# mkpython3/Mutation-Simulator

Hardware: AMD Instinct MI355X
Metric: Mbases mutated/sec on 3 Gb synthetic genome, ARGS SNP rate 0.01 (higher is better)
Workload: dtype u8

## Files before the change

include/msim.h:

```cpp
#ifndef MSIM_H
#define MSIM_H

#include <stdint.h>

#ifdef __cplusplus
extern "C" {
#endif

#define MSIM_ABI_VERSION 8

#define MSIM_OK               0
#define MSIM_ERR_ARG          1
#define MSIM_ERR_HIP          2
#define MSIM_ERR_VALUE        3
#define MSIM_ERR_KEY          4
#define MSIM_ERR_UNSUPPORTED  5
#define MSIM_ERR_NOMEM        6
#define MSIM_ERR_IO           7

#define MSIM_SN  1
#define MSIM_IN  2
#define MSIM_DE  3
#define MSIM_DU  4
#define MSIM_IV  5
// ... 182 lines not shown
#define MSIM_FASTA_HAS_BODY    1u
#define MSIM_FASTA_BAD_LINES   2u
#define MSIM_FASTA_NONUNIFORM  4u
typedef struct msim_fasta_record {
    uint64_t h0, h1;
    uint64_t b0, b1;
    uint64_t n_bases;
    uint32_t lenc, lenb;
    uint32_t flags, rsv;
} msim_fasta_record;
int msim_fasta_index(const uint8_t *text, uint64_t n, msim_fasta_record *records, uint64_t cap, uint64_t *n_records);

#define MSIM_COMM_ID_BYTES 128
int msim_comm_unique_id(uint8_t id[MSIM_COMM_ID_BYTES]);
int msim_comm_init(msim_ctx *ctx, const uint8_t id[MSIM_COMM_ID_BYTES], int rank, int world);
int msim_comm_destroy(msim_ctx *ctx);
int msim_planned_out_len(msim_ctx *ctx, int contig, uint64_t *out_len, int *known);
int msim_gather_to_root(msim_ctx *ctx, int n, const int *contig_ids, const int *owner, const uint64_t *out_len,
                        const uint64_t *n_records, const uint64_t *pool_len, int root, uint64_t *device_addrs);
int msim_gather_plan(int n, const int *owner, const uint64_t *out_len, const uint64_t *n_records, const uint64_t *pool_len,
                     int rank, int world, int root, int64_t *ops, int *n_ops);
int msim_gather_fetch(msim_ctx *ctx, uint64_t device_addr, uint64_t bytes, void *dst);

#define MSIM_SPECTRUM_TILE 4096
int msim_context_counts(msim_ctx *ctx, int contig, uint64_t counts[64], uint64_t *n_valid);
int msim_plan_contig_spectrum(msim_ctx *ctx, int contig, const uint64_t thr[192], uint64_t key, uint32_t seq);
int msim_spectrum_timing(msim_ctx *ctx, double *census_ms, double *plan_ms);
int msim_dbg_context_counts(const uint8_t *bases, uint64_t L, uint64_t counts[64], uint64_t *n_valid);
int msim_dbg_spectrum_plan(const uint8_t *bases, uint64_t L, const uint64_t thr[192], uint64_t key, uint32_t seq,
                           msim_record *recs, uint64_t cap, uint64_t *n_recs);
#define MSIM_SBS_CHANNELS 96
#define MSIM_SBS_TALLIES   8
#define MSIM_SBS_PASS   1024
int msim_sbs_counts(msim_ctx *ctx, int contig, uint64_t channels[96], uint64_t tallies[8]);
int msim_sbs_timing(msim_ctx *ctx, double *kernel_ms);
int msim_dbg_sbs_counts(const uint8_t *bases, uint64_t L, const msim_record *recs, uint64_t n_records,
                        uint64_t channels[96], uint64_t tallies[8]);

#define MSIM_CMP_EXACT  1u
#define MSIM_CMP_BINS   5
#define MSIM_CMP_PASS   256
#define MSIM_CMP_WINDOW 65536
int msim_cmp_hold(msim_ctx *ctx, int contig);
int msim_cmp_release(msim_ctx *ctx, int contig);
int msim_cmp_counts(msim_ctx *ctx, int contig, uint32_t flags, uint64_t *counts, uint64_t tallies[2]);
int msim_cmp_fetch(msim_ctx *ctx, int contig, uint64_t *n_held, uint64_t *held_pool_len, msim_record *held, uint8_t *held_pool,
                   uint8_t *held_flags, uint8_t *current_flags);
int msim_cmp_timing(msim_ctx *ctx, double *kernel_ms);
int msim_dbg_cmp_counts(const uint8_t *bases, uint64_t L, const msim_record *truth, uint64_t n_truth, const uint8_t *truth_pool,
                        uint64_t truth_pool_len, const msim_record *calls, uint64_t n_calls, const uint8_t *calls_pool,
                        uint64_t calls_pool_len, uint32_t flags, uint64_t *counts, uint64_t tallies[2], uint8_t *truth_flags,
                        uint8_t *calls_flags);

#define MSIM_CMP_BLOCK_GAP     50
#define MSIM_CMP_BLOCK_RECORDS 64
#define MSIM_CMP_BLOCK_SPAN    4096
int msim_cmp_counts_blocks(msim_ctx *ctx, int contig, uint32_t flags, uint32_t gap, uint64_t *counts, uint64_t tallies[2],
                           uint64_t block_tallies[5]);
int msim_cmp_blocks_timing(msim_ctx *ctx, double *kernel_ms);
int msim_dbg_cmp_counts_blocks(const uint8_t *bases, uint64_t L, const msim_record *truth, uint64_t n_truth, const uint8_t *truth_pool,
                               uint64_t truth_pool_len, const msim_record *calls, uint64_t n_calls, const uint8_t *calls_pool,
                               uint64_t calls_pool_len, uint32_t flags, uint32_t gap, uint64_t *counts, uint64_t tallies[2],
                               uint64_t block_tallies[5], uint8_t *truth_flags, uint8_t *calls_flags);

#define MSIM_CMP_TRUTH 0
#define MSIM_CMP_CALLS 1
#define MSIM_CMP_JOIN_TILE 1024
int msim_cmp_join(msim_ctx *ctx, int contig, int side);
int msim_cmp_counts_diploid(msim_ctx *ctx, int contig, uint32_t flags, uint64_t *counts, uint64_t tallies[2]);
int msim_cmp_fetch_diploid(msim_ctx *ctx, int contig, int side, uint64_t *n, uint64_t *pool_len, msim_record *recs, uint8_t *pool,
                           uint8_t *gt, uint8_t *flags);
int msim_cmp_join_timing(msim_ctx *ctx, double *kernel_ms);
int msim_dbg_cmp_join(const msim_record *h1, uint64_t n1, const uint8_t *pool1, uint64_t pool1_len, const msim_record *h2, uint64_t n2,
                      const uint8_t *pool2, uint64_t pool2_len, msim_record *out, uint8_t *out_pool, uint8_t *out_gt, uint64_t *n_out);
int msim_dbg_cmp_counts_diploid(const uint8_t *bases, uint64_t L, const msim_record *truth, uint64_t n_truth, const uint8_t *truth_pool,
                                uint64_t truth_pool_len, const uint8_t *truth_gt, const msim_record *calls, uint64_t n_calls,
                                const uint8_t *calls_pool, uint64_t calls_pool_len, const uint8_t *calls_gt, uint32_t flags,
                                uint64_t *counts, uint64_t tallies[2], uint8_t *truth_flags, uint8_t *calls_flags);

#define MSIM_SNP_BLOCK_WORDS 8192
int msim_dbg_snp_draws(msim_ctx *ctx, const uint32_t *words, uint64_t n_words, uint64_t ti_lim, uint64_t start, uint32_t K,
                       uint32_t aux_off, uint32_t *lanes, uint32_t *maps, uint64_t *end_pos, uint32_t *flags, uint8_t *aux);

int msim_stats(msim_ctx *ctx, msim_timing *out);
int msim_reset_stats(msim_ctx *ctx);

#ifdef __cplusplus
}
#endif
#endif
```

mutation-simulator_amd/csrc/apply.hip:

```cpp
#include <algorithm>
#include <vector>

#include "ctx.h"

#ifndef MSIM_ABL
#define MSIM_ABL 0
#endif

namespace msim {

namespace {

constexpr int THREADS = 256;
constexpr int GROUP = 16;
#ifndef MSIM_ITERS
#define MSIM_ITERS 4
#endif
constexpr int ITERS = MSIM_ITERS;
constexpr int TILE = THREADS * GROUP * ITERS;
constexpr int REC_CAP = 1024;
constexpr int REC_CAP_SMALL = 35 * ITERS;
constexpr int SCAN_ITEMS = 4;
constexpr int SCAN_BLOCK = THREADS * SCAN_ITEMS;

// ... 746 lines not shown
    } else {
        for (uint64_t i = i0; i < len; i++) dst[i] = (uint8_t)(w[(i - i0) >> 2] >> (((i - i0) & 3) * 8));
    }
}

__global__ __launch_bounds__(THREADS) void k_checksum(const uint8_t *__restrict__ src, uint64_t len,
                                                      unsigned long long *__restrict__ sum) {
    const uint64_t nwords = (len + 7) / 8;
    unsigned long long acc = 0;
    for (uint64_t k = (uint64_t)blockIdx.x * THREADS + threadIdx.x; k < nwords; k += (uint64_t)gridDim.x * THREADS) {
        uint64_t w;
        if (k * 8 + 8 <= len) {
            w = *reinterpret_cast<const uint64_t *>(src + k * 8);
        } else {
            w = 0;
            for (uint64_t i = k * 8; i < len; i++) w |= (uint64_t)src[i] << ((i - k * 8) * 8);
        }
        acc += mix64(w + k * 0x9E3779B97F4A7C15ull);
    }
    for (int o = 32; o > 0; o >>= 1) acc += __shfl_down(acc, o, 64);
    if ((threadIdx.x & 63) == 0) atomicAdd(sum, acc);
}

}

int dev_reserve(Ctx *c, DevBlock &b, size_t want_bytes) {
    if (b.raw && b.cap >= want_bytes) return MSIM_OK;
    MSIM_HIP(c, b.release());
    const size_t sz = want_bytes + (want_bytes >> 4) + 256;
    MSIM_HIP(c, dev_alloc(b, sz));
    return MSIM_OK;
}

int ensure_scratch(Ctx *c, size_t bytes) {
    DevBlock &b = c->d_scratch;
    if (bytes <= b.cap) return MSIM_OK;
    MSIM_HIP(c, wait_stream(c->stream));
    MSIM_HIP(c, wait_stream(c->emit_stream));
    MSIM_HIP(c, b.release());
    MSIM_HIP(c, dev_alloc(b, bytes + (bytes >> 2) + 4096));
    return MSIM_OK;
}

int synth_contig_device(Ctx *c, uint8_t *d_dst, uint64_t len, uint64_t seed) {
    if (len == 0) return MSIM_OK;
    const uint64_t lanes = (len + 31) / 32;
    const uint32_t blocks = (uint32_t)((lanes + THREADS - 1) / THREADS);
    hipLaunchKernelGGL(k_synth, dim3(blocks), dim3(THREADS), 0, c->stream, d_dst, len, seed);
    MSIM_HIP(c, hipGetLastError());
    return MSIM_OK;
}

int checksum_device(Ctx *c, const uint8_t *d_src, uint64_t len, uint64_t *sum) {
    int rc = ensure_scratch(c, 64);
    if (rc) return rc;
    unsigned long long *d_sum = reinterpret_cast<unsigned long long *>(c->d_scratch.raw);
    MSIM_HIP(c, hipMemsetAsync(d_sum, 0, 8, c->stream));
    if (len) {
        const uint64_t nwords = (len + 7) / 8;
        uint32_t blocks = (uint32_t)std::min<uint64_t>((nwords + THREADS - 1) / THREADS, 256 * 16);
        hipLaunchKernelGGL(k_checksum, dim3(blocks), dim3(THREADS), 0, c->stream, d_src, len, d_sum);
        MSIM_HIP(c, hipGetLastError());
    }
    unsigned long long h = 0;
    MSIM_HIP(c, hipMemcpyAsync(&h, d_sum, 8, hipMemcpyDeviceToHost, c->stream));
    MSIM_HIP(c, wait_stream(c->stream));
    *sum = h + len * 0x9E3779B97F4A7C15ull;
    return MSIM_OK;
}

extern uint8_t *ctx_lut(Ctx *c);

static int enqueue_err_copies(Ctx *c) {
    const size_t nc = c->contigs.size();
    if (c->h_errs.cap < 2 * nc * sizeof(unsigned long long)) {
        MSIM_HIP(c, c->h_errs.release());
        MSIM_HIP(c, pin_alloc(c->h_errs, (2 * nc + 64) * sizeof(unsigned long long)));
    }
    MSIM_HIP(c, hipMemcpyAsync(c->h_errs.p(), c->d_errs.p(), nc * sizeof(unsigned long long), hipMemcpyDeviceToHost, c->emit_stream));
    MSIM_HIP(c, hipMemcpyAsync(c->h_errs.p() + nc, c->d_errs.p() + MAX_CONTIGS, nc * sizeof(unsigned long long), hipMemcpyDeviceToHost, c->emit_stream));
    return MSIM_OK;
}

int apply_finish(Ctx *c) {
    bool have_errs = false;
    {
        int state = 0;
        const bool ride = c->fast && !c->pending_apply.empty();
        if (ride) {
            std::vector<hipStream_t> seen;
            for (auto it = c->pending_apply.rbegin(); it != c->pending_apply.rend(); ++it) {
                if (*it < 0 || (size_t)*it >= c->contigs.size()) continue;
                const Contig &g = c->contigs[(size_t)*it];
                hipStream_t s = g.apply_stream;
                if (!g.apply_pending || g.timing_shared || !g.ea2 || !s || s == c->emit_stream) continue;
                if (std::find(seen.begin(), seen.end(), s) != seen.end()) continue;
                seen.push_back(s);
                if (fast_lane_joined_at_collect(c, s)) continue;
                MSIM_HIP(c, hipStreamWaitEvent(c->emit_stream, g.ea2, 0));
            }
        }
        const int rc = fast_plan_collect(c, ride ? enqueue_err_copies : nullptr, &state);
        if (rc) { c->pending_apply.clear(); for (auto &g : c->contigs) g.apply_pending = g.dyn_applied = false; return rc; }
        have_errs = state == 1;
    }
    if (c->pending_apply.empty()) return MSIM_OK;
    {
        hipStream_t last = nullptr;
        for (int idx : c->pending_apply) {
            if (idx < 0 || (size_t)idx >= c->contigs.size()) continue;
            hipStream_t s = c->contigs[(size_t)idx].apply_stream;
            if (s && s != last && s != c->emit_stream) { MSIM_HIP(c, wait_stream(s)); last = s; }
        }
    }
    const size_t nc = c->contigs.size();
    if (!have_errs) {
        const int rc = enqueue_err_copies(c);
        if (rc) return rc;
        MSIM_HIP(c, wait_stream(c->emit_stream));
    }
    unsigned long long *errs = c->h_errs.p(), *deltas = c->h_errs.p() + nc;
    bool delta_mismatch = false;
    hipEvent_t origin = nullptr;
    std::vector<std::pair<float, float>> spans_all, spans_k;
    auto union_ms = [](std::vector<std::pair<float, float>> &v) {
        std::sort(v.begin(), v.end());
        double sum = 0;
        float lo = 0, hi = 0;
        bool open = false;
        for (const auto &iv : v) {
            if (open && iv.first <= hi) { hi = std::max(hi, iv.second); continue; }
            if (open) sum += hi - lo;
            lo = iv.first; hi = iv.second; open = true;
        }
        if (open) sum += hi - lo;
        return sum;
    };
    for (int idx : c->pending_apply) {
        if (idx < 0 || (size_t)idx >= c->contigs.size()) continue;
        Contig &g = c->contigs[(size_t)idx];
        if (!g.apply_pending) continue;
        g.apply_pending = false;
        if (g.dyn_applied) {
            g.dyn_applied = false;
            c->t.bytes_out += g.out_len;
            c->t.records += g.n_rec;
        }
        if (!g.timing_shared) {
            hipEvent_t e0 = g.ea0_is_ea1 ? g.ea1 : g.ea0;
            if (!origin) origin = e0;
            float t0 = 0, t1 = 0, t2 = 0;
            MSIM_HIP(c, hipEventElapsedTime(&t0, origin, e0));
            MSIM_HIP(c, hipEventElapsedTime(&t1, origin, g.ea1));
            MSIM_HIP(c, hipEventElapsedTime(&t2, origin, g.ea2));
            spans_all.push_back({t0, t2});
            spans_k.push_back({t1, t2});
        }
        g.timing_shared = false;
        const unsigned long long h_err = errs[(size_t)idx];
        g.key_error = h_err != ~0ull;
        if (g.key_error) { g.key_pos = h_err >> 8; g.key_base = (uint8_t)(h_err & 0xff); g.key_reported = false; }
        if (g.delta_known && !g.off_ready && !g.all_snp && g.n_rec && (long long)deltas[(size_t)idx] != g.known_delta) delta_mismatch = true;
    }
    c->pending_apply.clear();
    c->t.apply_ms += union_ms(spans_all);
    c->t.apply_kernel_ms += union_ms(spans_k);
    if (delta_mismatch) return fail(c, MSIM_ERR_HIP, "internal: planner and device disagree on the mutated length");
    return MSIM_OK;
}

struct RwPending { RwJob job; int variant; int contig; };

static_assert((TILE & (TILE - 1)) == 0, "the expansion's tile index shifts by log2(TILE)");
uint32_t apply_tile_shift() { return (uint32_t)__builtin_ctz((unsigned)TILE); }
int apply_prepare_tile_index(Ctx *c, Contig &g, hipStream_t st, int32_t **first, uint32_t *n_tiles, uint32_t *tile_shift,
                             unsigned long long **err) {
    const uint32_t nt = (uint32_t)((g.len + TILE - 1) / TILE);
    if (g.d_first.cap < (size_t)(nt + 1) * sizeof(int32_t)) MSIM_HIP(c, wait_stream(st));
    const int rc = dev_reserve(c, g.d_first, (size_t)(nt + 1) * sizeof(int32_t));
    if (rc) return rc;
    *first = g.d_first.p();
    *n_tiles = nt;
    *tile_shift = (uint32_t)__builtin_ctz((unsigned)TILE);
    *err = c->d_errs.p() + g.index;
    g.tile_index_by_plan = nt != 0;
    return MSIM_OK;
}

int apply_batch_device(Ctx *c, const std::vector<int> &ids, bool batch_rewrites) {
    TileJobs J;
    J.n_jobs = 0; J.total = 0;
    hipStream_t st = nullptr;
    auto launch = [&]() {
        if (J.n_jobs) hipLaunchKernelGGL(k_tile_index_batch, dim3((J.total + THREADS - 1) / THREADS), dim3(THREADS), 0, st, J);
        J.n_jobs = 0; J.total = 0;
    };
    std::vector<int> marked;
    int batch_first = -1;
    bool any_tile_job = false;
    for (int id : ids) {
        const Contig &g = c->contigs[(size_t)id];
        if (!(g.tile_index_by_plan && g.all_snp && !g.d_dyn)) any_tile_job = true;
    }
// ... 219 lines not shown
```

mutation-simulator_amd/csrc/ctx.h:

```cpp
#pragma once
#include <hip/hip_runtime.h>

#include <stdint.h>
#include <string>
#include <vector>

#include "../../include/msim.h"
#include "dev_block.h"
#include "mt19937.h"

namespace msim {

struct Contig {
    uint64_t len = 0;
    Scratch<uint8_t> d_in;
    bool planned = false;
    bool plan_empty = true;
    bool all_snp = false;
    bool delta_known = false;
    long long known_delta = 0;
    bool off_ready = false;
    const uint32_t *d_dyn = nullptr;
    bool sizes_pending = false;
    bool dyn_applied = false;
// ... 2 lines not shown
    uint64_t n_struct_est = 0;
    hipStream_t apply_stream = nullptr;
    Scratch<int32_t> d_first;
    bool tile_index_done = false;
    bool tile_index_by_plan = false;
    bool timing_shared = false;
    uint64_t n_rec = 0, pool_len = 0;
    Scratch<msim_record> d_recs;
    Scratch<uint8_t> d_pool;
    bool applied = false;
    uint64_t out_len = 0;
    Scratch<uint8_t> d_out;
    Scratch<uint32_t> d_off;
    uint8_t key_base = 0;
    uint64_t key_pos = 0;
    bool key_error = false;
    bool key_reported = false;
    int index = 0;
    bool apply_pending = false;
    bool defer_apply = false;
    hipEvent_t ea0 = nullptr, ea1 = nullptr, ea2 = nullptr;
    bool ea0_is_ea1 = false;
    std::vector<msim_record> h_recs;
    std::vector<uint8_t> h_pool;
    std::vector<uint8_t> h_in;
    bool have_gt = false;
    Scratch<uint8_t> d_gt;
    std::vector<uint8_t> h_gt;
    int hap = 0;
    Scratch<msim_record> d_recs_hap;
    struct FullTable {
        Scratch<msim_record> d_recs;
        uint64_t n_rec = 0;
        bool all_snp = false, delta_known = false;
        long long known_delta = 0;
        std::vector<msim_record> h_recs;
    } full;
};

constexpr uint64_t PAD = 64;

struct GpuPlan;
struct FastPlan;
struct Comm;
struct Batch;
struct FileIo;
struct VcfState;
struct SpectrumState;
struct CompareState;

struct Ctx {
    int device = 0;
    bool host_only = false;
    bool chain_only = false;
    uint32_t flags = 0;
    hipStream_t stream = nullptr;
    hipStream_t emit_stream = nullptr;
    hipEvent_t ev0 = nullptr, ev1 = nullptr, ev2 = nullptr, ev3 = nullptr;
    std::string err;
    std::string devname;
    HostMT py, np;
    GpuPlan *gpu = nullptr;
    Comm *comm = nullptr;
    void *rw_collect = nullptr;
    Batch *batch = nullptr;
    FileIo *file_io = nullptr;
    VcfState *vcf = nullptr;
    SpectrumState *spectrum = nullptr;
    CompareState *compare = nullptr;
    msim_params params{};
    bool have_params = false;
    std::vector<Contig> contigs;
    int deferred_apply = -1;
    int deferred_more[3] = {-1, -1, -1};
    int n_deferred_more = 0;
    uint64_t fast_key = 0x9E3779B97F4A7C15ull;
    uint32_t fast_seq = 0;
    FastPlan *fast = nullptr;
    msim_timing t{};
    DevBlock d_scratch;
    Pinned<unsigned long long> h_mail;
    Scratch<unsigned long long> d_errs;
    Pinned<unsigned long long> h_errs;
    std::vector<int> pending_apply;
    Scratch<uint8_t> d_text;
    uint64_t text_len = 0;
    int text_contig = -1, text_kind = 0;
    uint32_t text_bpl = 0;
    uint64_t text_chain_id = 0;
    std::string text_chain_names;
    double chain_kernel_ms = -1.0;
    Scratch<uint8_t> d_text_scratch;
};

struct TraceRange {
    explicit TraceRange(const char *name);
    ~TraceRange();
    TraceRange(const TraceRange &) = delete;
    TraceRange &operator=(const TraceRange &) = delete;
    bool on;
};

int fail(Ctx *c, int code, const std::string &msg);
int hip_fail(Ctx *c, hipError_t e, const char *what);

constexpr hipError_t MSIM_WAIT_TIMED_OUT = hipErrorLaunchTimeOut;
hipError_t wait_stream(hipStream_t s);
hipError_t wait_event(hipEvent_t ev);
double wait_limit_seconds();

#define MSIM_HIP(ctx, call)                                              \
    do {                                                                 \
        hipError_t e__ = (call);                                         \
        if (e__ != hipSuccess) return ::msim::hip_fail((ctx), e__, #call); \
    } while (0)

int flush_deferred_apply(Ctx *c, bool only_groups = false);
bool deferred_apply_holds(const Ctx *c, int contig);

int ctx_flush_queued(Ctx *c);
#define CTX_FLUSHED(c, p)                                   \
    ::msim::Ctx *c = reinterpret_cast<::msim::Ctx *>(p);    \
    if (c) {                                                \
        const int flush_rc_ = ::msim::ctx_flush_queued(c);  \
        if (flush_rc_) return flush_rc_;                    \
    }
int ctx_device_contig(Ctx *c, int contig, bool need_planned, Contig **out);

struct EventPair {
    hipEvent_t e0 = nullptr, e1 = nullptr;
    hipError_t create() { const hipError_t e = hipEventCreate(&e0); return e != hipSuccess ? e : hipEventCreate(&e1); }
    void destroy() {
        if (e0) (void)hipEventDestroy(e0);
        if (e1) (void)hipEventDestroy(e1);
        e0 = e1 = nullptr;
    }
    hipError_t begin(hipStream_t s) const { return hipEventRecord(e0, s); }
    hipError_t end(hipStream_t s) const { return hipEventRecord(e1, s); }
    int add_elapsed(Ctx *c, double *acc) const {
        float ms = 0;
        MSIM_HIP(c, hipEventElapsedTime(&ms, e0, e1));
        *acc += ms;
        return MSIM_OK;
    }
};
struct CopySource { const void *src; size_t bytes; };
int copy_floor(Ctx *c, const EventPair &tm, const CopySource *srcs, int n_srcs, double *ms);

template <class T> __host__ __device__ __forceinline__ void rec_lengths(const msim_record &r, T &outlen, T &inlen) {
    const T len = (T)r.stop - (T)r.pos + 1;
    switch (r.type) {
        case MSIM_SN: outlen = 1; inlen = 1; break;
        case MSIM_IN: outlen = len + 1; inlen = 1; break;
        case MSIM_DE: outlen = 0; inlen = len; break;
        case MSIM_IV: outlen = len; inlen = len; break;
        case MSIM_DU: outlen = 2 * len; inlen = len; break;
        case MSIM_TL: outlen = 0; inlen = len; break;
        case MSIM_TLI: {
            const T ilen = (T)r.stop + 1 > (T)r.extra ? (T)r.stop + 1 - (T)r.extra : 0;
            outlen = ilen + 1; inlen = 1; break;
        }
        default: outlen = 0; inlen = 0; break;
    }
}
inline long long rec_delta(const msim_record &r) {
    long long outlen, inlen;
// ... 66 lines not shown
    static bool types_ok(const uint8_t *type, size_t n, bool with_tl = false);
    void run(const uint32_t *pos, const uint8_t *type, size_t n, const uint32_t *T, size_t w_lim, uint32_t *stop);
    void run_tl(const uint32_t *pos, const uint8_t *type, size_t n, const uint32_t *T, size_t w_lim, uint32_t *stop);
    int finish(Ctx *c, size_t n, size_t *consumed) const;
};
int chain_boundary_tables(Ctx *c, const msim_range &r, uint64_t L, const uint32_t *pos, const uint8_t *type, size_t n,
                          const ChainClasses &cc, const uint32_t *T, size_t n_words, uint32_t *stop, size_t *consumed,
                          size_t *kept, long long *len_delta);

struct WordFeed { int (*more)(void *user, size_t *avail); void *user; };
int cut_ranges_host(Ctx *c, const msim_range *ranges, int n_ranges, int64_t d, const uint32_t *words, size_t n_words,
                    uint32_t *cut, uint32_t *pool_pos, size_t *n_pool_pos, size_t *consumed, const WordFeed *feed = nullptr);

int sample_ranges_host(Ctx *c, const msim_range *ranges, int n_ranges, int64_t d, const uint32_t *words,
                       size_t n_words, uint32_t *pos_out, size_t *consumed);

struct MixSets {
    ChainClasses gcc{};
    std::vector<uint32_t> set_of;
    std::vector<int> rep;
    std::vector<ChainClasses> cc;
    bool sn_chained = false;
    bool has_tl = false;
    uint64_t K = 0;
    uint32_t n_draw = 0;
};
bool multimix_prepare(const Ctx *c, uint64_t L, const msim_range *ranges, int n_ranges, MixSets &ms);
constexpr uint8_t CHAIN_TOMBSTONE = 0x80;
int multimix_walk_host(Ctx *c, uint64_t L, const msim_range *ranges, int n_ranges, int64_t d, const MixSets &ms,
                       const uint32_t *words, const uint32_t *T, size_t n_words, const uint32_t *ch_rank,
                       const uint8_t *ch_type, size_t n_ch, uint32_t *cand_pos, uint32_t *ch_stop, uint32_t *visit_from,
                       size_t *consumed, const WordFeed *feed = nullptr, uint32_t *ch_extra = nullptr,
                       uint8_t *ch_aux = nullptr);
int link_translocations(Ctx *c, const uint32_t *words, size_t n_words, const uint32_t *ch_pos, const uint8_t *ch_type,
                        uint32_t *ch_stop, uint32_t *ch_extra, uint8_t *ch_aux, size_t n_ch, size_t *consumed);
void count_translocations(const uint8_t *type, const uint32_t *stop, size_t n, size_t *n_tl, size_t *n_tli);
int multimix_plan_emulated(Ctx *c, uint64_t L, const msim_range *ranges, int n_ranges, HostPlan &out);

struct FastPlan;
void fast_plan_destroy(Ctx *c);
int fast_plan_check(Ctx *c, uint64_t L, const msim_range *ranges, int n_ranges);
int plan_contig_fast(Ctx *c, Contig &ct, const msim_range *ranges, int n_ranges, uint64_t key, uint32_t seq);
int fast_plan_flush(Ctx *c);
bool fast_plan_queued(Ctx *c, int contig, bool mark_apply);
int fast_plan_collect(Ctx *c, int (*behind)(Ctx *) = nullptr, int *behind_state = nullptr);
bool fast_lane_joined_at_collect(const Ctx *c, hipStream_t s);
int fast_plan_emulated(Ctx *c, uint64_t L, const msim_range *ranges, int n_ranges, uint64_t key, uint32_t seq, HostPlan &out);

int vcf_render_device(Ctx *c, Contig &g, const char *seq_name, uint64_t *bytes, DevBlock *into = nullptr);
int chain_render_device(Ctx *c, Contig &g, const char *t_name, const char *q_name, uint64_t id, double *kernel_ms = nullptr);
uint32_t chain_tile();
int fasta_frame_device(Ctx *c, Contig &g, uint32_t bpl, uint64_t *bytes, DevBlock *into = nullptr);
int splice_device(Ctx *c, const Contig &a, const Contig *b, const uint32_t *seg_out, const uint32_t *seg_src, uint32_t n_seg,
                  Contig &dst);
int fasta_gather_device(Ctx *c, const uint8_t *body, uint64_t body_bytes, uint64_t n_bases, uint32_t lenc,
                        uint32_t lenb, uint8_t *d_dst);

int file_check(Ctx *c, int fd);
int file_text_buffer(Ctx *c, int ch, int *slot, DevBlock **buf);
int file_enqueue(Ctx *c, int ch, int slot, uint64_t n, int fd, uint64_t offset);
int file_enqueue_host(Ctx *c, int ch, const uint8_t *src, uint64_t n, int fd, uint64_t offset);
void file_channel_idle(Ctx *c, int ch);
int file_wait(Ctx *c);
void file_io_destroy(Ctx *c);
int file_bgzf_open(Ctx *c, int ch, int fd);
int file_bgzf_append(Ctx *c, int ch, const uint8_t *src, uint64_t n);
int file_bgzf_close(Ctx *c, int ch, uint64_t *compressed, uint64_t *uncompressed);
uint64_t bgzf_bound(uint64_t n);
int bgzf_compress_host(Ctx *c, const uint8_t *src, uint64_t n, uint8_t *out, uint64_t cap, uint64_t *written, float *device_ms);
int bgzf_probe_host(const uint8_t *src, uint64_t n, uint64_t *uncompressed, uint64_t *members);
int bgzf_inflate_host(Ctx *c, const uint8_t *src, uint64_t n, uint8_t *out, uint64_t cap, uint64_t *written, float *device_ms);
void device_host_cpus(int device, char *buf, size_t cap);

uint64_t render_vcf_unchecked(const msim_record *recs, uint64_t n_records, const uint8_t *insert_pool, const uint8_t *bases,
                              uint64_t len, const char *seq_name, char *out);
void chain_header(char *out, uint64_t *n, uint64_t L, uint64_t sum_dt, uint64_t sum_dq, uint64_t t_start, uint64_t q_start,
                  uint64_t t_trail, uint64_t q_trail, const char *t_name, const char *q_name, uint64_t id);

void comm_destroy(Ctx *c);

int apply_contig_device(Ctx *c, Contig &g);
int apply_batch_device(Ctx *c, const std::vector<int> &ids, bool batch_rewrites);
int apply_finish(Ctx *c);
uint32_t apply_tile_shift();
int apply_prepare_tile_index(Ctx *c, Contig &g, hipStream_t st, int32_t **first, uint32_t *n_tiles, uint32_t *tile_shift,
                             unsigned long long **err);
constexpr int MAX_CONTIGS = 1 << 16;
int synth_contig_device(Ctx *c, uint8_t *d_dst, uint64_t len, uint64_t seed);
int checksum_device(Ctx *c, const uint8_t *d_src, uint64_t len, uint64_t *sum);
int ensure_scratch(Ctx *c, size_t bytes);
int dev_reserve(Ctx *c, DevBlock &b, size_t want_bytes);

}
```

mutation-simulator_amd/csrc/msim_api.hip:

```cpp
#include <algorithm>
#include <chrono>
#include <cstdio>
#include <cstring>
#include <new>
#include <thread>

#include <dlfcn.h>

#include "ctx.h"
#include "plan_gpu.h"

namespace msim {

static thread_local std::string g_create_error;

namespace {
struct Roctx {
    int (*push)(const char *) = nullptr;
    int (*pop)() = nullptr;
    Roctx() {
        for (const char *n : {"librocprofiler-sdk-roctx.so.1", "libroctx64.so.4", "libroctx64.so"}) {
            void *h = dlopen(n, RTLD_NOW | RTLD_GLOBAL);
            if (!h) continue;
            *reinterpret_cast<void **>(&push) = dlsym(h, "roctxRangePushA");
            *reinterpret_cast<void **>(&pop) = dlsym(h, "roctxRangePop");
            if (push && pop) return;
            push = nullptr; pop = nullptr;
        }
    }
};
Roctx &roctx() { static Roctx r; return r; }
}

TraceRange::TraceRange(const char *name) : on(false) {
    Roctx &r = roctx();
    if (r.push) { (void)r.push(name); on = true; }
}
TraceRange::~TraceRange() { if (on) (void)roctx().pop(); }

int fail(Ctx *c, int code, const std::string &msg) {
    if (c) c->err = msg; else g_create_error = msg;
    return code;
}
int hip_fail(Ctx *c, hipError_t e, const char *what) {
    if (e == MSIM_WAIT_TIMED_OUT) {
        char buf[160];
        snprintf(buf, sizeof buf, ": no completion within %g s (MSIM_WAIT_TIMEOUT_S); the work it waits for is still queued or the device hangs",
                 wait_limit_seconds());
        return fail(c, MSIM_ERR_HIP, std::string(what) + buf);
    }
    return fail(c, MSIM_ERR_HIP, std::string(what) + ": " + hipGetErrorString(e));
}

double wait_limit_seconds() {
    const char *e = getenv("MSIM_WAIT_TIMEOUT_S");
    if (!e || !*e) return 120.0;
    const double v = atof(e);
    return v > 0 ? v : 0.0;
}

template <class Q>
static hipError_t wait_poll(Q &&query) {
    hipError_t e = query();
    if (e != hipErrorNotReady) return e;
    const auto t0 = std::chrono::steady_clock::now();
    for (;;) {
        for (int i = 0; i < 16; i++) __builtin_ia32_pause();
        if ((e = query()) != hipErrorNotReady) return e;
        if (std::chrono::steady_clock::now() - t0 > std::chrono::milliseconds(2)) break;
    }
    const double limit = wait_limit_seconds();
    for (;;) {
        std::this_thread::sleep_for(std::chrono::microseconds(50));
        if ((e = query()) != hipErrorNotReady) return e;
        if (limit > 0 && std::chrono::duration<double>(std::chrono::steady_clock::now() - t0).count() > limit) return MSIM_WAIT_TIMED_OUT;
    }
}
hipError_t wait_stream(hipStream_t s) { return wait_poll([s]() { return hipStreamQuery(s); }); }
hipError_t wait_event(hipEvent_t ev) { return wait_poll([ev]() { return hipEventQuery(ev); }); }

struct CtxDev {
    Scratch<uint8_t> d_lut;
};
static CtxDev *dev_of(Ctx *c);
uint8_t *ctx_lut(Ctx *c) { return dev_of(c)->d_lut.p(); }

static int drain(Ctx *c);
int ctx_drain(Ctx *c) { return drain(c); }
static int drain(Ctx *c) {
    if (c->host_only) return MSIM_OK;
    TraceRange tr("msim drain (collect deferred results)");
    int rc = c->gpu ? gpu_plan_finish(c, c->gpu) : MSIM_OK;
    int rc2 = apply_finish(c);
    if (rc) return rc;
    if (rc2) return rc2;
    MSIM_HIP(c, wait_stream(c->stream));
    MSIM_HIP(c, wait_stream(c->emit_stream));
    return MSIM_OK;
}
static int defer_group_size() {
    static const int n = getenv("MSIM_NO_DEFER_PAIRS") ? 1 : getenv("MSIM_DEFER_GROUP") ? std::min(4, std::max(1, atoi(getenv("MSIM_DEFER_GROUP")))) : 3;
    return n;
}
bool deferred_apply_holds(const Ctx *c, int contig) {
    if (c->deferred_apply == contig) return contig >= 0;
    for (int q = 0; q < c->n_deferred_more; q++) if (c->deferred_more[q] == contig) return true;
    return false;
}
int flush_deferred_apply(Ctx *c, bool only_groups) {
    if (c->deferred_apply < 0) return MSIM_OK;
    if (only_groups && c->n_deferred_more + 1 < defer_group_size()) return MSIM_OK;
    std::vector<int> ids;
    for (int q = 0; q < c->n_deferred_more; q++) ids.push_back(c->deferred_more[q]);
    ids.push_back(c->deferred_apply);
    c->deferred_apply = -1;
    c->n_deferred_more = 0;
    ids.erase(std::remove_if(ids.begin(), ids.end(), [&](int idx) { return idx < 0 || idx >= (int)c->contigs.size(); }), ids.end());
    if (ids.size() >= 2) {
        for (int idx : ids) c->contigs[(size_t)idx].apply_stream = c->emit_stream;
        return apply_batch_device(c, ids, true);
    }
    for (int idx : ids) {
        const int rc = apply_contig_device(c, c->contigs[(size_t)idx]);
        if (rc) return rc;
    }
    return MSIM_OK;
}
int ctx_flush_queued(Ctx *c) {
    int rc = flush_deferred_apply(c);
    if (!rc && c->fast) rc = fast_plan_flush(c);
    if (!rc && c->gpu) rc = gpu_emit_flush(c);
    return rc;
}
int ctx_device_contig(Ctx *c, int contig, bool need_planned, Contig **out) {
    int rc = ctx_flush_queued(c);
    if (rc) return rc;
    if (c->host_only) return fail(c, MSIM_ERR_HIP, "host-only context: this call needs the GPU");
    if (contig < 0 || (size_t)contig >= c->contigs.size()) return fail(c, MSIM_ERR_ARG, "no such contig");
    Contig &g = c->contigs[(size_t)contig];
    if (need_planned) {
        if (!g.planned) return fail(c, MSIM_ERR_ARG, "contig has not been planned");
        if ((rc = ctx_drain(c))) return rc;
    }
    *out = &g;
    return MSIM_OK;
}
int copy_floor(Ctx *c, const EventPair &tm, const CopySource *srcs, int n_srcs, double *ms) {
    *ms = 0;
    size_t total = 0;
    for (int i = 0; i < n_srcs; i++) total += srcs[i].bytes;
    if (!total) return MSIM_OK;
    const int rc = ensure_scratch(c, total);
    if (rc) return rc;
    MSIM_HIP(c, tm.begin(c->stream));
    uint8_t *dst = (uint8_t *)c->d_scratch.raw;
    for (int i = 0; i < n_srcs; dst += srcs[i++].bytes)
        if (srcs[i].bytes) MSIM_HIP(c, hipMemcpyAsync(dst, srcs[i].src, srcs[i].bytes, hipMemcpyDeviceToDevice, c->stream));
    MSIM_HIP(c, tm.end(c->stream));
    MSIM_HIP(c, wait_stream(c->stream));
    return tm.add_elapsed(c, ms);
}
static int key_error_of(Ctx *c, Contig &g) {
    g.key_reported = true;
    return fail(c, MSIM_ERR_KEY, std::string("KeyError: '") + (char)g.key_base + "'");
}

struct CtxFull : Ctx { CtxDev dev; };
static CtxDev *dev_of(Ctx *c) { return &static_cast<CtxFull *>(c)->dev; }

static void build_lut(uint8_t *lut) {
    uint8_t conv[256], comp[256], ti[256];
    for (int i = 0; i < 256; i++) conv[i] = comp[i] = ti[i] = (uint8_t)i;
    const char *a = "KSYMWRBDHV-", *b = "GCCAAACAAAN";
    for (int i = 0; a[i]; i++) conv[(uint8_t)a[i]] = (uint8_t)b[i];
    a = "ACGTUMRWSYKVHDB"; b = "TGCAAKYWSRMBDHV";
// ... 1140 lines not shown
        if (o < 0 || o >= (1ll << 32)) return bad(i, "output offset outside [0, 2^32)");
        if (off) (*off)[(size_t)i] = (uint32_t)o;
        run += d;
        next_free = last + 1;
    }
    const long long out_len = (long long)L + run;
    if (out_len < 0 || out_len >= (1ll << 32)) return fail(c, MSIM_ERR_ARG, "mutated length outside [0, 2^32)");
    *delta = run;
    return MSIM_OK;
}

int msim_dbg_set_records(msim_ctx *p, int contig, const msim_record *recs, uint64_t n_records, const uint8_t *insert_pool,
                         uint64_t pool_len, uint32_t flags) {
    CTX_FLUSHED(c, p)
    if (!c || (n_records && !recs) || (pool_len && !insert_pool) || (flags & ~1u)) return MSIM_ERR_ARG;
    Contig *g = get_contig(c, contig);
    if (!g) return MSIM_ERR_ARG;
    const bool with_offsets = flags & 1u;
    std::vector<uint32_t> off;
    long long delta = 0;
    int rc = check_record_table(c, g->len, recs, n_records, pool_len, with_offsets ? &off : nullptr, &delta);
    if (rc) return rc;
    if ((rc = drain(c))) return rc;
    reset_contig(*g);
    c->text_kind = 0;
    g->apply_stream = nullptr;
    std::vector<msim_record> rv(recs, recs + n_records);
    std::vector<uint8_t> pv(insert_pool, insert_pool + pool_len);
    if ((rc = install_host_table(c, g, rv, pv, n_records == 0))) return rc;
    if (!with_offsets) return MSIM_OK;
    g->delta_known = true;
    g->known_delta = delta;
    if (c->host_only || g->all_snp || !n_records) return MSIM_OK;
    rc = dev_reserve(c, g->d_off, (size_t)n_records * sizeof(uint32_t));
    if (rc) return rc;
    MSIM_HIP(c, hipMemcpyAsync(g->d_off.p(), off.data(), (size_t)n_records * sizeof(uint32_t), hipMemcpyHostToDevice, c->stream));
    MSIM_HIP(c, wait_stream(c->stream));
    g->off_ready = true;
    return MSIM_OK;
}

int msim_dbg_apply_batch(msim_ctx *p, const int *contigs, int n) {
    CTX_FLUSHED(c, p)
    if (!c || !contigs || n < 1) return MSIM_ERR_ARG;
    NEED_GPU(c);
    std::vector<int> ids(contigs, contigs + n);
    for (int i = 0; i < n; i++) {
        Contig *g = get_contig(c, ids[(size_t)i]);
        if (!g) return MSIM_ERR_ARG;
        if (!g->planned || g->d_dyn || !(g->all_snp || (g->off_ready && g->delta_known)))
            return fail(c, MSIM_ERR_ARG, "msim_dbg_apply_batch: a contig without a table installed with its offsets");
        for (int q = 0; q < i; q++) if (ids[(size_t)q] == ids[(size_t)i]) return fail(c, MSIM_ERR_ARG, "msim_dbg_apply_batch: contig listed twice");
    }
    int rc = drain(c);
    if (rc) return rc;
    c->text_kind = 0;
    for (int id : ids) c->contigs[(size_t)id].apply_stream = c->emit_stream;
    return apply_batch_device(c, ids, true);
}

uint32_t msim_dbg_apply_tile(void) { return 1u << apply_tile_shift(); }
int msim_dbg_emit_train(msim_ctx *p, int n_jobs, const uint64_t *const *bitmaps, const uint32_t *n_words, const uint32_t *start,
                        const uint64_t *contig_len, const uint8_t *const *aux8, uint32_t d, int train, msim_record *const *recs,
                        const uint64_t *cap_recs, uint64_t *n_recs, int32_t *const *first) {
    CTX_FLUSHED(c, p)
    if (!c) return MSIM_ERR_ARG;
    NEED_GPU(c);
    int rc = drain(c);
    if (rc) return rc;
    return gpu_dbg_emit_train(c, n_jobs, bitmaps, n_words, start, contig_len, aux8, d, train, apply_tile_shift(), recs, cap_recs,
                              n_recs, first);
}

int msim_dbg_snp_draws(msim_ctx *p, const uint32_t *words, uint64_t n_words, uint64_t ti_lim, uint64_t start, uint32_t K,
                       uint32_t aux_off, uint32_t *lanes, uint32_t *maps, uint64_t *end_pos, uint32_t *flags, uint8_t *aux) {
    CTX_FLUSHED(c, p)
    if (!c) return MSIM_ERR_ARG;
    NEED_GPU(c);
    int rc = drain(c);
    if (rc) return rc;
    return gpu_dbg_snp_draws(c, words, n_words, ti_lim, start, K, aux_off, lanes, maps, end_pos, flags, aux);
}

int msim_dbg_candidates(msim_ctx *p, const uint64_t *bitmap, uint32_t n_words, uint32_t start, uint32_t d, uint32_t K,
                        const void *rt, uint32_t n_draw, const void *sets, uint32_t n_sets, const uint32_t *np_words, uint64_t n_np_words,
                        uint32_t all, uint32_t *cand_pos, uint8_t *cand_type, uint32_t *nsn_pos, uint8_t *nsn_type, uint32_t *nsn_rank,
                        uint64_t cap, uint32_t *k_out, uint32_t *n_nsn) {
    CTX_FLUSHED(c, p)
    if (!c) return MSIM_ERR_ARG;
    NEED_GPU(c);
    int rc = drain(c);
    if (rc) return rc;
    return gpu_dbg_candidates(c, bitmap, n_words, start, d, K, rt, n_draw,
                              sets, n_sets, np_words, n_np_words, all, cand_pos, cand_type, nsn_pos,
                              nsn_type, nsn_rank, cap, k_out, n_nsn);
}

int msim_dbg_accept_tables(msim_ctx *p, const uint32_t *raw_words, uint64_t n_words, uint64_t p0, uint32_t n, const uint32_t *shift,
                           const uint32_t *width, uint32_t n_classes, uint32_t *T, uint32_t *T_ps) {
    CTX_FLUSHED(c, p)
    if (!c) return MSIM_ERR_ARG;
    NEED_GPU(c);
    int rc = drain(c);
    if (rc) return rc;
    return gpu_dbg_accept_tables(c, raw_words, n_words, p0, n, shift, width, n_classes, T, T_ps);
}

int msim_dbg_accept_tables_host(const uint32_t *tempered, uint32_t n, const uint32_t *shift, const uint32_t *width, uint32_t n_classes,
                                uint32_t *T) {
    ChainClasses cc;
    if (!T || (n && !tempered) || n > (1u << 26) || !dbg_chain_classes(shift, width, n_classes, cc)) return MSIM_ERR_ARG;
    memset(T, 0, (((size_t)n + 1) << chain_lg_rows(cc)) * 4);
    accept_tables_host(cc, tempered, n, T);
    return MSIM_OK;
}

int msim_dbg_mixed_emit(msim_ctx *p, uint64_t L, uint32_t k, const uint32_t *cand_pos, const uint8_t *cand_type, uint32_t n_ch,
                        const uint32_t *ch_rank, const uint32_t *ch_stop, const uint32_t *ch_extra, const uint8_t *ch_aux, uint32_t n_draw,
                        const void *rt, const uint32_t *visit_from, uint32_t sn_chained, const uint32_t *np_words, uint64_t n_np_words,
                        msim_record *recs, uint32_t *rec_off, uint32_t *sn_index, uint8_t *pool, uint64_t cap_pool, uint32_t *counts,
                        int64_t *len_delta) {
    CTX_FLUSHED(c, p)
    if (!c) return MSIM_ERR_ARG;
    NEED_GPU(c);
    int rc = drain(c);
    if (rc) return rc;
    return gpu_dbg_mixed_emit(c, L, k, cand_pos, cand_type, n_ch, ch_rank, ch_stop, ch_extra, ch_aux, n_draw,
                              rt, visit_from, sn_chained, np_words, n_np_words, recs, rec_off, sn_index,
                              pool, cap_pool, counts, len_delta);
}

int msim_dbg_stream_moments(uint64_t n, uint64_t k, uint64_t K, uint64_t ti_lim, double out[4]) {
    if (!out || !n || k >= n) return MSIM_ERR_ARG;
    const StreamMoments a = sample_words_moments(n, k), b = snp_words_moments(K, (unsigned long long)ti_lim);
    out[0] = a.e; out[1] = a.v; out[2] = b.e; out[3] = b.v;
    return MSIM_OK;
}

int msim_dbg_stream_need(const msim_params *params, const msim_range *ranges, int n_ranges, double out[7]) {
    if (!params || !ranges || n_ranges < 1 || !out) return MSIM_ERR_ARG;
    const msim_range &r = ranges[0];
    const double n = (double)range_population(r, min_block(*params)), k = (double)r.k;
    if (n < 1) return MSIM_ERR_ARG;
    const StreamNeed need = stream_need(*params, ranges, n_ranges);
    const StreamMoments m = small_sample_moments(n, k, (double)r.setsize);
    out[0] = need.py; out[1] = need.np; out[2] = need.bad ? 1.0 : 0.0;
    out[3] = big_sample_window(n, set_path_need(n, k)); out[4] = m.e; out[5] = m.v; out[6] = randint_acceptance_min(r);
    return MSIM_OK;
}

int msim_dbg_stream_status(msim_ctx *p, int out[8]) {
    CTX_FLUSHED(c, p)
    if (!c || !out || c->host_only || !c->gpu) return MSIM_ERR_ARG;
    gpu_plan_stream_status(c, c->gpu, out);
    return MSIM_OK;
}

__global__ void k_dbg_stall(unsigned long long ticks) {
    const unsigned long long t0 = wall_clock64();
    while (wall_clock64() - t0 < ticks) __builtin_amdgcn_s_sleep(127);
}
int msim_dbg_stall(msim_ctx *p, int which, uint32_t ms) {
    Ctx *c = C(p);
    if (!c || c->host_only || which < 0 || which > 1 || ms > 10000) return MSIM_ERR_ARG;
    hipLaunchKernelGGL(k_dbg_stall, dim3(1), dim3(1), 0, which ? c->emit_stream : c->stream, (unsigned long long)ms * 100000ull);
    MSIM_HIP(c, hipGetLastError());
// ... 72 lines not shown
```

mutation-simulator_amd/csrc/plan_gpu.h:

```cpp
#pragma once
#include "ctx.h"
#include "plan_windows.h"

namespace msim {

struct GpuPlan;
GpuPlan *gpu_plan_create();
void gpu_plan_destroy(GpuPlan *g);
void gpu_plan_invalidate(GpuPlan *g);
int gpu_plan_sync_to_host(Ctx *c, GpuPlan *g);
void gpu_plan_reserve(GpuPlan *g, uint64_t py_words, uint64_t np_words);
int gpu_plan_finish(Ctx *c, GpuPlan *g);
bool gpu_plan_eligible(const Ctx *c, const msim_range *ranges, int n_ranges);
int plan_contig_gpu(Ctx *c, GpuPlan *g, Contig &ct, const msim_range *ranges, int n_ranges);
bool gpu_plan_mixed_eligible(const Ctx *c, const msim_range *ranges, int n_ranges);
int plan_contig_gpu_mixed(Ctx *c, GpuPlan *g, Contig &ct, const msim_range *ranges, int n_ranges);
bool gpu_plan_hostsample_eligible(const Ctx *c, const msim_range *ranges, int n_ranges);
int plan_contig_gpu_hostsample(Ctx *c, GpuPlan *g, Contig &ct, const msim_range *ranges, int n_ranges);
bool gpu_plan_multimix_eligible(const Ctx *c, GpuPlan *g, uint64_t L, const msim_range *ranges, int n_ranges);
int plan_contig_gpu_multimix(Ctx *c, GpuPlan *g, Contig &ct, const msim_range *ranges, int n_ranges);
int gpu_emit_flush(Ctx *c);
bool gpu_emit_pending(Ctx *c, int contig, bool mark_apply);
int gpu_dbg_emit_train(Ctx *c, int n_jobs, const uint64_t *const *bm, const uint32_t *n_words, const uint32_t *start,
                       const uint64_t *len, const uint8_t *const *aux8, uint32_t d, int train, uint32_t tile_shift,
                       msim_record *const *recs, const uint64_t *cap_recs, uint64_t *n_recs, int32_t *const *first);
int gpu_dbg_snp_draws(Ctx *c, const uint32_t *words, uint64_t n_words, uint64_t ti_lim, uint64_t start, uint32_t K, uint32_t aux_off,
                      uint32_t *lanes, uint32_t *maps, uint64_t *end_pos, uint32_t *flags, uint8_t *aux);
int gpu_dbg_candidates(Ctx *c, const uint64_t *bm, uint32_t n_words, uint32_t start, uint32_t d, uint32_t K, const void *rt,
                       uint32_t n_draw, const void *sets, uint32_t n_sets, const uint32_t *np_raw, uint64_t n_np, uint32_t all,
                       uint32_t *cand_pos, uint8_t *cand_type, uint32_t *nsn_pos, uint8_t *nsn_type, uint32_t *nsn_rank, uint64_t cap,
                       uint32_t *k_out, uint32_t *n_nsn);
int gpu_dbg_accept_tables(Ctx *c, const uint32_t *raw, uint64_t n_words, uint64_t p0, uint32_t n, const uint32_t *sh,
                          const uint32_t *width, uint32_t n_classes, uint32_t *T, uint32_t *T_ps);
int gpu_dbg_mixed_emit(Ctx *c, uint64_t L, uint32_t k, const uint32_t *cand_pos, const uint8_t *cand_type, uint32_t n_ch,
                       const uint32_t *ch_rank, const uint32_t *ch_stop, const uint32_t *ch_extra, const uint8_t *ch_aux,
                       uint32_t n_draw, const void *rt, const uint32_t *visit_from, uint32_t sn_chained, const uint32_t *np_raw,
                       uint64_t n_np, msim_record *recs, uint32_t *rec_off, uint32_t *sn_index, uint8_t *pool, uint64_t cap_pool,
                       uint32_t *counts, int64_t *len_delta);
int gpu_plan_force_overflow(Ctx *c, GpuPlan *g);
void gpu_plan_abandon(GpuPlan *g);
int gpu_plan_make_room(Ctx *c, GpuPlan *g, const msim_range *ranges, int n_ranges, bool *fits);
struct StreamNeed { double py, np; bool bad; };
StreamNeed stream_need(const msim_params &P, const msim_range *ranges, int n_ranges);

void gpu_plan_stream_status(Ctx *c, GpuPlan *g, int out[8]);

StreamMoments sample_words_moments(uint64_t n, uint64_t k);
StreamMoments snp_words_moments(uint64_t K, unsigned long long ti_lim);

}
```

mutation-simulator_amd/csrc/plan_gpu.hip:

```cpp
#include <algorithm>
#include <chrono>
#include <cmath>
#include <cstdio>
#include <cstdlib>
#include <cstring>
#include <vector>
#include <sys/mman.h>

#include "ctx.h"
#include "mt_jump_table.h"
#include "plan_gpu.h"
#include "plan_kernels.h"

namespace msim {

struct GpuStream {
    uint32_t *d_raw = nullptr;
    uint64_t cap = 0;
    uint32_t *d_states = nullptr;
    uint32_t states_cap = 0;
    uint32_t n_states = 0;
    uint32_t lvl = 0, n_src = 1, m_done = 0;
    SnpMap *d_maps = nullptr;
    SnpLane *d_lanes = nullptr;
// ... 13 lines not shown
    uint32_t waited_words = 0;
    hipEvent_t casc_ev = nullptr;
    bool casc_pending = false;
    std::vector<hipEvent_t> ready_ev;
    uint32_t waited_chunks = 0;
};

static hipError_t host_stage_free(void *p);
using PinBlock = Block<host_stage_free>;
template <class T> struct Staging : PinBlock { T *p() const { return static_cast<T *>(raw); } };

constexpr int N_SETS = 32;

struct SampleSet {
    Scratch<uint32_t> acc;
    Scratch<uint32_t> cnt;
    Scratch<uint32_t> bitmap;
    Scratch<uint32_t> cnt2;
    Scratch<uint32_t> bins;
    Scratch<uint32_t> cursors;
    uint8_t *ahead = nullptr;
    Scratch<uint32_t> hcnt, hacc;
    hipEvent_t prep_done = nullptr;
    hipEvent_t chain_done = nullptr;
    uint8_t last_user = 0;
    hipEvent_t emit_done = nullptr;
    hipEvent_t wait_ev = nullptr;
    bool pending = false;
};
struct SnpSet {
    Scratch<SnpMap> maps;
    Scratch<uint8_t> aux8;
    unsigned long long *base = nullptr;
    hipEvent_t emit_done = nullptr;
    hipEvent_t wait_ev = nullptr;
    bool pending = false;
};

struct SnpDefer { SnpSet *T; uint32_t W2, nb2; };
struct EmitItem { int contig; SampleSet *S; SnpSet *T; uint32_t bmw, bnb, start, K, W2, nb2; msim_record *recs; bool apply; };

struct MixedSet {
    Scratch<uint32_t> cand_pos;
    Scratch<uint8_t> cand_type;
    Scratch<uint32_t> cand_stop;
    Scratch<uint32_t> nsn_pos;
    Scratch<uint8_t> nsn_type;
    Scratch<uint32_t> nsn_rank;
    Scratch<uint32_t> nsn_stop;
    Scratch<uint32_t> sn_index;
    Scratch<uint32_t> cnt;
    Scratch<uint32_t> words;
    unsigned long long *p0_slot = nullptr;
    Scratch<WalkRange> walk_d;
    Staging<WalkRange> walk_h;
    Scratch<uint32_t> wbits;
    bool wbits_dirty = false;
    Scratch<uint32_t> wcnt;
    Scratch<uint32_t> tables;
    Scratch<uint32_t> cand_extra;
    Scratch<uint8_t> cand_aux;
    Scratch<uint32_t> nsn_extra;
    Scratch<uint8_t> nsn_aux;
    Scratch<uint8_t> mm_d;
    Staging<uint8_t> mm_h;
    hipEvent_t emit_done = nullptr;
    bool pending = false;
};

struct GpuPlan {
    GpuStream s[2];
    MixedSet mixed[N_SETS];
    uint32_t mixed_unit = 0;
    Staging<uint32_t> h_words;
    Staging<uint32_t> h_npos;
    Staging<uint8_t> h_ntype;
    Staging<uint32_t> h_nstop;
    Staging<uint32_t> h_win;
    Staging<uint32_t> h_nrank;
    Staging<uint32_t> h_nextra;
    Staging<uint8_t> h_naux;
    MixSets mm_sets;
    const msim_range *mm_for = nullptr; int mm_n = 0;
    uint32_t *h_seed = nullptr;
    hipEvent_t seed_ev[2] = {nullptr, nullptr};
    hipStream_t gen_stream = nullptr;
    hipStream_t jump_stream = nullptr;
    std::vector<hipEvent_t> ev_pool;
    uint32_t *d_poly = nullptr;
    PlanState *d_ps = nullptr;
    PlanState *h_mail = nullptr;
    uint32_t *h_sig = nullptr;
    uint32_t epoch = 0;
    hipStream_t copy_stream = nullptr;
    hipEvent_t ev_cand = nullptr, ev_piece[3] = {}, ev_cpiece[3] = {};
    SampleSet sample[N_SETS];
    SnpSet snp[N_SETS];
    uint32_t unit = 0, snp_unit = 0;
    hipEvent_t chain_ev[2 * N_SETS] = {};
    uint32_t chain_i = 0;
    hipEvent_t grp_ev[2 * N_SETS] = {};
    uint32_t grp_i = 0;
    hipEvent_t t0 = nullptr, t1 = nullptr;
    bool ps_valid = false;
    bool unverified = false;
    std::vector<EmitItem> emit_items;
    uint32_t emit_d = 1;
    uint64_t verified_pos = 0;
    uint64_t reserve_words[2] = {0, 0};
    int emit_group = 0;
    int emit_train = 0;
    uint32_t max_chunks = MT_JUMP_MAX_CHUNKS;
    uint32_t rebases = 0;
    uint32_t cand_cap = 0xffffffffu;
    hipStream_t prep_stream = nullptr;
    hipStream_t prep_streams[8] = {};
    int n_prep = 4, n_prep_low = 1, prep_i = 0, prep_prio = 0;
    double ahead_sigma = 8.0;
    uint32_t prep_waited[8] = {};
    int ahead = 2;
    uint32_t pass_chain_only = 0;
    bool sharded_rank = false;
    bool est_ok = false;
    double est_e = 0, est_v = 0;
    uint64_t est_lo = 0;
};

GpuPlan *gpu_plan_create() {
    GpuPlan *g = new GpuPlan();
    if (const char *e = getenv("MSIM_EMIT_GROUP")) g->emit_group = std::min(EMIT_G, std::max(0, atoi(e)));
    if (const char *e = getenv("MSIM_DBG_JUMP_MAX_CHUNKS"))
        g->max_chunks = (uint32_t)std::min<long>(MT_JUMP_MAX_CHUNKS, std::max<long>(2, atol(e)));
    if (const char *e = getenv("MSIM_DBG_CAND_CAP")) g->cand_cap = (uint32_t)std::min<long>(0xffffffffl, std::max<long>(1, atol(e)));
    if (const char *e = getenv("MSIM_EMIT_TRAIN")) g->emit_train = atoi(e) == 3 ? 3 : atoi(e) == 6 ? 6 : 0;
    if (getenv("MSIM_NO_AHEAD")) g->ahead = 0;
    else if (const char *e = getenv("MSIM_AHEAD")) g->ahead = std::min(2, std::max(0, atoi(e)));
    if (const char *e = getenv("MSIM_PREP_STREAMS")) { g->n_prep = std::min(8, std::max(1, atoi(e))); g->n_prep_low = 0; }
    if (const char *e = getenv("MSIM_PREP_LOW")) g->n_prep_low = std::min(g->n_prep, std::max(0, atoi(e)));
    if (const char *e = getenv("MSIM_PREP_PRIO")) g->prep_prio = atoi(e);
    if (const char *e = getenv("MSIM_AHEAD_SIGMA")) g->ahead_sigma = std::min(16.0, std::max(0.0, atof(e)));
    return g;
}

constexpr size_t STAGE_HUGE = (size_t)2 << 20;
static void *host_stage_alloc(size_t sz, hipError_t *err) {
    *err = hipSuccess;
    const size_t total = sz + 2 * STAGE_HUGE;
    void *raw = mmap(nullptr, total, PROT_READ | PROT_WRITE, MAP_PRIVATE | MAP_ANONYMOUS, -1, 0);
    if (raw == MAP_FAILED) return nullptr;
    uint8_t *q = reinterpret_cast<uint8_t *>(((uintptr_t)raw + STAGE_HUGE + STAGE_HUGE - 1) & ~(uintptr_t)(STAGE_HUGE - 1));
    size_t *hdr = reinterpret_cast<size_t *>(q - 4096);
    hdr[0] = (size_t)(uintptr_t)raw;
    hdr[1] = total;
#ifdef MADV_HUGEPAGE
    (void)madvise(q, sz, MADV_HUGEPAGE);
#endif
    *err = hipHostRegister(q, sz, hipHostRegisterDefault);
    if (*err != hipSuccess) { munmap(raw, total); return nullptr; }
    return q;
}
static hipError_t host_stage_free(void *p) {
    (void)hipDeviceSynchronize();
    const hipError_t e = hipHostUnregister(p);
    const size_t *hdr = reinterpret_cast<const size_t *>(static_cast<uint8_t *>(p) - 4096);
    munmap(reinterpret_cast<void *>((uintptr_t)hdr[0]), hdr[1]);
    return e;
}

// ... 7 lines not shown
            MSIM_HIP(c, wait_stream(c->stream));
            MSIM_HIP(c, wait_stream(c->emit_stream));
            grew = true;
        }
        MSIM_HIP(c, b.release());
        const size_t sz = want_bytes + want_bytes / 4 + 4096;
        MSIM_HIP(c, hipMalloc(&b.raw, sz));
        b.cap = sz;
        return MSIM_OK;
    }
    int own(PinBlock &b, size_t want_bytes) {
        if (b.cap >= want_bytes) return MSIM_OK;
        (void)b.release();
        const size_t sz = (want_bytes + want_bytes / 4 + STAGE_HUGE) & ~(STAGE_HUGE - 1);
        hipError_t e;
        void *q = host_stage_alloc(sz, &e);
        if (!q) return e != hipSuccess ? hip_fail(c, e, "hipHostRegister(host staging buffer)") : fail(c, MSIM_ERR_NOMEM, "host staging buffer");
        b.raw = q;
        b.cap = sz;
        return MSIM_OK;
    }
    struct Want { PinBlock &b; size_t bytes; };
    int shared(std::initializer_list<Want> group) {
        bool waited = false;
        for (const Want &w : group) {
            if (w.b.cap >= w.bytes) continue;
            if (!waited) {
                MSIM_HIP(c, wait_stream(c->stream));
                if (c->gpu && c->gpu->copy_stream) MSIM_HIP(c, wait_stream(c->gpu->copy_stream));
                waited = true;
            }
            if (int rc = own(w.b, w.bytes)) return rc;
        }
        return MSIM_OK;
    }
};

struct DbgDev {
    std::vector<DevBlock> blocks;
    template <class T> hipError_t bytes(T **out, size_t sz) {
        void *q = nullptr;
        const hipError_t e = hipMalloc(&q, sz);
        if (e == hipSuccess) { blocks.emplace_back(); blocks.back().raw = q; }
        *out = static_cast<T *>(q);
        return e;
    }
    template <class T> hipError_t get(T **out, size_t n) { return bytes(out, std::max<size_t>(n * sizeof(T), 4) + PAD); }
};

void gpu_plan_destroy(GpuPlan *g) {
    if (!g) return;
    if (g->jump_stream) { (void)wait_stream(g->jump_stream); (void)hipStreamDestroy(g->jump_stream); }
    if (g->gen_stream) { (void)wait_stream(g->gen_stream); (void)hipStreamDestroy(g->gen_stream); }
    for (auto st : g->prep_streams) if (st) { (void)wait_stream(st); (void)hipStreamDestroy(st); }
    for (auto &s : g->s) {
        if (s.d_raw) (void)hipFree(s.d_raw);
        if (s.d_states) (void)hipFree(s.d_states);
        if (s.d_z) (void)hipFree(s.d_z);
        if (s.d_maps) (void)hipFree(s.d_maps);
        if (s.d_lanes) (void)hipFree(s.d_lanes);
        for (auto e : s.ready_ev) (void)hipEventDestroy(e);
        for (auto e : s.words_ev) if (e) (void)hipEventDestroy(e);
        if (s.casc_ev) (void)hipEventDestroy(s.casc_ev);
    }
    for (auto e : g->ev_pool) (void)hipEventDestroy(e);
    for (auto &t : g->sample) {
        if (t.ahead) (void)hipFree(t.ahead);
        if (t.prep_done) (void)hipEventDestroy(t.prep_done);
        if (t.chain_done) (void)hipEventDestroy(t.chain_done);
        if (t.emit_done) (void)hipEventDestroy(t.emit_done);
    }
    for (auto &t : g->snp) {
        if (t.base) (void)hipFree(t.base);
        if (t.emit_done) (void)hipEventDestroy(t.emit_done);
    }
    for (auto &t : g->mixed) {
        if (t.p0_slot) (void)hipFree(t.p0_slot);
        if (t.emit_done) (void)hipEventDestroy(t.emit_done);
    }
    for (auto e : g->chain_ev) if (e) (void)hipEventDestroy(e);
    for (auto e : g->grp_ev) if (e) (void)hipEventDestroy(e);
    if (g->t0) (void)hipEventDestroy(g->t0);
    if (g->t1) (void)hipEventDestroy(g->t1);
    if (g->h_seed) (void)hipHostFree(g->h_seed);
    for (auto e : g->seed_ev) if (e) (void)hipEventDestroy(e);
    if (g->d_poly) (void)hipFree(g->d_poly);
    if (g->d_ps) (void)hipFree(g->d_ps);
    if (g->h_mail) (void)hipHostFree(g->h_mail);
    if (g->h_sig) (void)hipHostFree(g->h_sig);
    if (g->copy_stream) (void)hipStreamDestroy(g->copy_stream);
    if (g->ev_cand) (void)hipEventDestroy(g->ev_cand);
    for (auto e : g->ev_cpiece) if (e) (void)hipEventDestroy(e);
    for (auto e : g->ev_piece) if (e) (void)hipEventDestroy(e);
    delete g;
}

void gpu_plan_invalidate(GpuPlan *g) {
    g->unit = g->snp_unit = g->mixed_unit = 0;
    g->sharded_rank = g->pass_chain_only > 0;
    g->pass_chain_only = 0;
    for (auto &s : g->s) {
        if (s.live) s.last_session_words = std::max<uint64_t>(s.pos, s.max_upto);
        s.live = false;
    }
}
void gpu_plan_reserve(GpuPlan *g, uint64_t py_words, uint64_t np_words) { g->reserve_words[0] = py_words; g->reserve_words[1] = np_words; }

static inline uint64_t span_words(const GpuPlan *g) { return (uint64_t)MT_N + (uint64_t)g->max_chunks * MT_CHUNK_WORDS; }

StreamNeed stream_need(const msim_params &P, const msim_range *ranges, int n_ranges) {
    const int64_t d = min_block(P);
    double py = 0, K = 0, K_chain = 0, pool_mean = 0, pool_var = 0, e_small = 0, var_small = 0;
    bool has_tl = false, bad = false;
    int n_big = 0;
    for (int i = 0; i < n_ranges; i++) {
        const msim_range &r = ranges[i];
        if (r.k <= 0) continue;
        const double k = (double)r.k, n = (double)range_population(r, d);
        const bool pool = n <= (double)r.setsize;
        K += k;
        if (n < k || (!pool && n >= 4294967296.0)) bad = true;
        else if (!pool && r.k >= 4096) {
            py += big_sample_window(n, set_path_need_bounded(n, k));
            n_big++;
        } else {
            const StreamMoments m = small_sample_moments(n, k, (double)r.setsize);
            e_small += m.e; var_small += m.v;
        }
        bool chain = P.block[MSIM_SN] != d;
        for (int j = 0; j < r.n_types; j++) {
            const int t = r.types[j];
            if (t == MSIM_SN || !type_drawable(r, j)) continue;
            chain = true;
            if (t == MSIM_TL || t == MSIM_TLI) has_tl = true;
            if (t == MSIM_IN) {
                const double q = type_probability(r, j);
                const double mx = (double)std::max<int64_t>(r.max_len[t], 1);
                pool_mean += k * q * mx;
                pool_var += k * q * mx * mx;
            }
        }
        if (chain) K_chain += k;
    }
    py += e_small + 16.0 * std::sqrt(var_small);
    if (K_chain > 0) py += randint_window(K_chain, 0.5);
    if (has_tl) py += 6.0 * K_chain + 16.0 * std::sqrt(25.0 * K_chain + 1.0) + 4096.0;
    py += 4.0 * K + 16.0 * std::sqrt(4.0 * K) + 16384.0 + 3.0 * SNP_BLOCK2;
    py += 2.0 * 65536.0 + 8192.0 * n_big;
    return StreamNeed{py, 2.0 * K + pool_mean + 16.0 * std::sqrt(pool_var) + 4096.0, bad};
}

int gpu_plan_make_room(Ctx *c, GpuPlan *g, const msim_range *ranges, int n_ranges, bool *fits) {
    const StreamNeed need = stream_need(c->params, ranges, n_ranges);
    const double py = need.py, np = need.np, span = (double)(span_words(g) - MT_N);
    *fits = need.bad || (std::isfinite(py) && py < span && np < span);
    if (need.bad || !*fits) return MSIM_OK;
    const GpuStream &s0 = g->s[0], &s1 = g->s[1];
    const bool live = s0.live || s1.live;
    const double at0 = s0.live ? (double)s0.pos : (double)MT_N, at1 = s1.live ? (double)s1.pos : (double)MT_N;
    if (live && (at0 + py > (double)span_words(g) || at1 + np > (double)span_words(g))) {
        const int rc = gpu_plan_sync_to_host(c, g);
        if (rc) return rc;
        g->rebases++;
        c->t.stream_rebases++;
    }
    return MSIM_OK;
}

// ... 118 lines not shown
                    if (rc) return rc;
                    MSIM_HIP(c, hipEventRecord(wev, gs));
                    if (first) {
                        MSIM_HIP(c, hipStreamWaitEvent(g->gen_stream, wev, 0));
                        s.waited_words = hi;
                    }
                }
                if (si == 0) {
                    const uint32_t n_words = (uint32_t)(MT_N + (uint64_t)hi * MT_CHUNK_WORDS);
                    const uint32_t complete = n_words / SNP_BLOCK2;
                    if (complete > s.mapped_blocks) {
                        hipLaunchKernelGGL(k_snp_maps_abs, dim3(complete - s.mapped_blocks), dim3(SNP_THREADS), 0, g->gen_stream,
                                           s.d_raw, n_words, (unsigned long long)c->params.ti_lim, s.mapped_blocks, s.d_maps, s.d_lanes);
                        MSIM_HIP(c, hipGetLastError());
                        s.mapped_blocks = complete;
                    }
                }
                hipEvent_t ev;
                rc = take_event(ev);
                if (rc) return rc;
                MSIM_HIP(c, hipEventRecord(ev, g->gen_stream));
                s.ready_hi.push_back(hi);
                s.ready_ev.push_back(ev);
                s.words_ev.push_back(wev);
                s.n_chunks = hi;
            }
            if (s.n_chunks < need_chunks) {
                if (s.m_done == (uint32_t)MT_JUMP_RADIX[s.lvl] - 1) {
                    s.lvl++;
                    s.n_src = s.n_states;
                    s.m_done = 0;
                }
                const uint32_t R = (uint32_t)MT_JUMP_RADIX[s.lvl];
                const uint32_t m_need = std::min<uint32_t>(R - 1, (need_chunks + s.n_src - 1) / s.n_src - 1);
                uint32_t level_base = 0;
                for (uint32_t l = 0; l < s.lvl; l++) level_base += (uint32_t)MT_JUMP_RADIX[l] - 1;
                const bool on_plan = lead_on_plan && s.lvl <= 1 && s.n_chunks == 0;
                hipStream_t js = on_plan ? c->stream : g->jump_stream;
                if (!on_plan) { const int rcj = join_plan_cascade(); if (rcj) return rcj; }
                if (s.z_lvl != (int)s.lvl) {
                    if (s.z_cap < s.n_src) {
                        MSIM_HIP(c, wait_stream(g->jump_stream));
                        MSIM_HIP(c, wait_stream(c->stream));
                        if (s.d_z) MSIM_HIP(c, hipFree(s.d_z));
                        s.d_z = nullptr; s.z_cap = 0;
                        MSIM_HIP(c, hipMalloc(&s.d_z, (size_t)s.n_src * JUMP_ZP * sizeof(uint32_t)));
                        s.z_cap = s.n_src;
                    }
                    hipLaunchKernelGGL(k_mt_extend, dim3(s.n_src), dim3(GEN_THREADS), 0, js, s.d_states, s.d_z);
                    MSIM_HIP(c, hipGetLastError());
                    s.z_lvl = (int)s.lvl;
                }
                hipLaunchKernelGGL(k_mt_jump, dim3(s.n_src * (m_need - s.m_done)), dim3(JUMP_THREADS), 0,
                                   js, s.d_states, s.d_z, s.n_src,
                                   g->d_poly + (size_t)level_base * MT_POLY_WORDS, s.m_done + 1);
                MSIM_HIP(c, hipGetLastError());
                if (on_plan) {
                    if (!s.casc_ev) MSIM_HIP(c, hipEventCreateWithFlags(&s.casc_ev, hipEventDisableTiming));
                    MSIM_HIP(c, hipEventRecord(s.casc_ev, c->stream));
                    s.casc_pending = true;
                }
                s.m_done = m_need;
                s.n_states = s.n_src * (s.m_done + 1);
            }
        }
    }
    if (upto > MT_N) {
        const uint32_t need = (uint32_t)((upto - MT_N + MT_CHUNK_WORDS - 1) / MT_CHUNK_WORDS);
        if (need > (maps ? s.waited_chunks : s.waited_words)) {
            for (size_t b = 0; b < s.ready_hi.size(); b++) {
                if (s.ready_hi[b] >= need) {
                    const bool words_only = !maps && s.words_ev[b];
                    MSIM_HIP(c, hipStreamWaitEvent(c->stream, words_only ? s.words_ev[b] : s.ready_ev[b], 0));
                    s.waited_words = std::max(s.waited_words, s.ready_hi[b]);
                    if (!words_only) s.waited_chunks = s.ready_hi[b];
                    break;
                }
            }
        }
    }
    return MSIM_OK;
}

static int stream_to_device(Ctx *c, GpuPlan *g, int si) {
    GpuStream &s = g->s[si];
    HostMT &h = si ? c->np : c->py;
    if (s.live) return MSIM_OK;
    if (!s.d_states) {
        MSIM_HIP(c, hipMalloc(&s.d_states, (size_t)MT_N * sizeof(uint32_t)));
        s.states_cap = 1;
    }
    if (!s.d_raw) {
        MSIM_HIP(c, hipMalloc(&s.d_raw, (size_t)MT_N * sizeof(uint32_t)));
        s.cap = MT_N;
    }
    {
        int rc0 = ensure_side_streams(c, g);
        if (rc0) return rc0;
    }
    MSIM_HIP(c, wait_stream(g->jump_stream));
    MSIM_HIP(c, wait_stream(g->gen_stream));
    for (auto st : g->prep_streams) if (st) MSIM_HIP(c, wait_stream(st));
    if (!g->h_seed) MSIM_HIP(c, hipHostMalloc(&g->h_seed, 2 * sizeof h.mt, hipHostMallocDefault));
    if (!g->seed_ev[si]) MSIM_HIP(c, hipEventCreateWithFlags(&g->seed_ev[si], hipEventDisableTiming));
    else MSIM_HIP(c, wait_event(g->seed_ev[si]));
    uint32_t *slot = g->h_seed + (size_t)si * MT_N;
    memcpy(slot, h.mt, sizeof h.mt);
    MSIM_HIP(c, hipMemcpyAsync(s.d_states, slot, sizeof h.mt, hipMemcpyHostToDevice, c->stream));
    MSIM_HIP(c, hipMemcpyAsync(s.d_raw, slot, sizeof h.mt, hipMemcpyHostToDevice, c->stream));
    MSIM_HIP(c, hipEventRecord(g->seed_ev[si], c->stream));
    MSIM_HIP(c, hipStreamWaitEvent(g->jump_stream, g->seed_ev[si], 0));
    MSIM_HIP(c, hipStreamWaitEvent(g->gen_stream, g->seed_ev[si], 0));
    if (si == 0) for (auto st : g->prep_streams) if (st) MSIM_HIP(c, hipStreamWaitEvent(st, g->seed_ev[si], 0));
    for (auto e : s.ready_ev) g->ev_pool.push_back(e);
    s.ready_ev.clear();
    s.ready_hi.clear();
    for (auto e : s.words_ev) if (e) g->ev_pool.push_back(e);
    s.words_ev.clear();
    s.waited_chunks = 0;
    s.waited_words = 0;
    if (si == 0) for (auto &w : g->prep_waited) w = 0;
    s.casc_pending = false;
    s.n_states = 1;
    s.lvl = 0; s.n_src = 1; s.m_done = 0;
    s.z_lvl = -1;
    s.n_chunks = 0;
    s.mapped_blocks = 0;
    s.maps_ti_lim = c->params.ti_lim;
    s.pos = (uint64_t)h.idx;
    s.max_upto = 0;
    s.live = true;
    if (si == 0) { g->ps_valid = false; g->verified_pos = s.pos; }
    return MSIM_OK;
}

static int session_open(Ctx *c, GpuPlan *g) {
    int rc;
    if ((rc = stream_to_device(c, g, 0))) return rc;
    if ((rc = stream_to_device(c, g, 1))) return rc;
    if (!g->d_ps) MSIM_HIP(c, hipMalloc(&g->d_ps, sizeof(PlanState)));
    if (!g->h_mail) MSIM_HIP(c, hipHostMalloc(&g->h_mail, sizeof(PlanState), hipHostMallocMapped));
    return MSIM_OK;
}
static int chain_open(Ctx *c, GpuPlan *g, bool sampler) {
    if (!g->t0) { MSIM_HIP(c, hipEventCreate(&g->t0)); MSIM_HIP(c, hipEventCreate(&g->t1)); }
    if (!g->unverified) MSIM_HIP(c, hipEventRecord(g->t0, c->stream));
    if (!g->ps_valid) {
        hipLaunchKernelGGL(k_state_init, dim3(1), dim3(1), 0, c->stream, g->d_ps, (unsigned long long)g->s[0].pos);
        g->ps_valid = true;
    }
    if (!sampler) { g->unverified = true; g->est_ok = false; }
    return MSIM_OK;
}

int gpu_plan_sync_to_host(Ctx *c, GpuPlan *g) {
    int frc = gpu_plan_finish(c, g);
    if (frc) return frc;
    for (int si = 0; si < 2; si++) {
        GpuStream &s = g->s[si];
        if (!s.live) continue;
        HostMT &h = si ? c->np : c->py;
        const uint64_t consumed = s.pos;
        int rc = ensure_words(c, g, si, consumed);
        if (rc) return rc;
        if (consumed >= MT_N) {
            MSIM_HIP(c, hipMemcpyAsync(h.mt, s.d_raw + (consumed - MT_N), sizeof h.mt, hipMemcpyDeviceToHost, c->stream));
            h.idx = MT_N;
        } else {
            MSIM_HIP(c, hipMemcpyAsync(h.mt, s.d_raw, sizeof h.mt, hipMemcpyDeviceToHost, c->stream));
            h.idx = (int)consumed;
        }
        MSIM_HIP(c, wait_stream(c->stream));
        h.state_changed();
        s.last_session_words = std::max<uint64_t>(s.pos, s.max_upto);
        s.live = false;
    }
    return MSIM_OK;
}

bool gpu_plan_eligible(const Ctx *c, const msim_range *ranges, int n_ranges) {
    const msim_params &P = c->params;
    const int64_t d = min_block(P);
    if (P.block[MSIM_SN] != d) return false;
    int64_t prev_stop = -1;
    for (int i = 0; i < n_ranges; i++) {
        const msim_range &r = ranges[i];
        if (r.k == 0) continue;
        if (r.k < 4096) return false;
        if (r.start <= prev_stop) return false;
        prev_stop = r.stop;
        const int64_t n = range_population(r, d);
        if (r.k < 0 || n < r.k) return false;
        if (n <= r.setsize || n >= (1ll << 32)) return false;
        if (r.start < 0 || r.stop >= (1ll << 32)) return false;
        if (!range_is_deterministic_sn(r)) return false;
    }
    return true;
}

int gpu_plan_finish(Ctx *c, GpuPlan *g) {
    {
        const int rc = gpu_emit_flush(c);
        if (rc) return rc;
    }
    if (!g->unverified) return MSIM_OK;
    hipLaunchKernelGGL(k_publish, dim3(1), dim3(1), 0, c->stream, g->d_ps, g->h_mail);
    MSIM_HIP(c, hipGetLastError());
    MSIM_HIP(c, hipEventRecord(g->t1, c->stream));
    MSIM_HIP(c, wait_stream(c->stream));
    MSIM_HIP(c, wait_stream(c->emit_stream));
    float ms = 0;
    MSIM_HIP(c, hipEventElapsedTime(&ms, g->t0, g->t1));
    c->t.plan_gpu_ms += ms;
    g->unverified = false;
    for (auto &t : g->sample) { t.pending = false; t.last_user = 0; }
    for (auto &t : g->snp) t.pending = false;
    for (auto &t : g->mixed) t.pending = false;
    const PlanState h = *g->h_mail;
    if (h.flags & (FLAG_SAMPLE_OVERFLOW | FLAG_SNP_OVERFLOW)) {
        g->s[0].live = g->s[1].live = false;
        for (auto &t : g->mixed) t.wbits_dirty = true;
        return fail(c, MSIM_ERR_HIP, "GPU sampler: a stream window overflowed its margin (16 sigma; 8 for the start of a sample planned ahead of the chain; results discarded)");
    }
    c->t.py_words += h.pos - g->verified_pos;
    c->t.snp_ahead_margin_permille = std::max<uint64_t>(c->t.snp_ahead_margin_permille, h.ahead_margin_used);
    g->verified_pos = h.pos;
    g->s[0].pos = h.pos;
    return MSIM_OK;
}

void gpu_plan_abandon(GpuPlan *g) {
    g->s[0].live = g->s[1].live = false;
    g->unverified = false;
    g->ps_valid = false;
    g->est_ok = false;
}

int gpu_plan_force_overflow(Ctx *c, GpuPlan *g) {
    if (!g->d_ps) return MSIM_OK;
    hipLaunchKernelGGL(k_raise_flag, dim3(1), dim3(1), 0, c->stream, g->d_ps, (uint32_t)FLAG_SAMPLE_OVERFLOW);
    MSIM_HIP(c, hipGetLastError());
    g->unverified = true;
    return MSIM_OK;
}

static hipEvent_t next_chain_event(GpuPlan *g) {
    hipEvent_t &e = g->chain_ev[g->chain_i++ % (2 * N_SETS)];
    if (!e) (void)hipEventCreateWithFlags(&e, hipEventDisableTiming);
    return e;
}

static int wait_if_pending(Ctx *c, bool &pending, hipEvent_t ev) {
    if (!pending) return MSIM_OK;
    if (hipEventQuery(ev) == hipSuccess) { pending = false; return MSIM_OK; }
    (void)hipGetLastError();
    MSIM_HIP(c, hipStreamWaitEvent(c->stream, ev, 0));
    return MSIM_OK;
}

static uint32_t sample_bin_cap(uint64_t n, uint32_t k, double p_acc) {
    const uint32_t nbk = (uint32_t)((double)k / p_acc / SPL_BLOCK) + 3;
    const double mean = (double)((nbk + BIN_SUBS - 1) / BIN_SUBS) * SPL_BLOCK * p_acc * std::min(1.0, (double)BIN_VALUES / (double)n);
    return (uint32_t)std::min<double>((double)k + 16.0, 1.25 * mean + 16.0 * std::sqrt(mean) + 512.0);
}

struct SampleLaunch { SampleSet *S; uint32_t W, bmw, bnb; };
static int enqueue_sample_chain(Ctx *c, GpuPlan *g, const msim_range &r, int64_t d, uint64_t pos_hi, Grow &grow,
                                SampleLaunch &out, const uint32_t *raw_other = nullptr, PlanState *ps_other = nullptr,
                                uint64_t e_limit = ~0ull) {
    const uint32_t *raw = raw_other ? raw_other : g->s[0].d_raw;
    PlanState *ps = ps_other ? ps_other : g->d_ps;
    int rc;
    const uint32_t k = (uint32_t)r.k;
    const uint64_t n = (uint64_t)range_population(r, d);
    const int bits = bit_length64(n);
    const double p_acc = randbelow_acceptance((double)n);
    const double wd = big_sample_window((double)n, set_path_need((double)n, (double)k));
    if (wd >= 4.0e9) return fail(c, MSIM_ERR_UNSUPPORTED, "sample window beyond 2^32 words");
    const uint32_t W = (uint32_t)wd;
    SampleSet &S = g->sample[g->unit++ % N_SETS];
    S.last_user = 1;
    if ((rc = wait_if_pending(c, S.pending, S.wait_ev))) return rc;
    const uint32_t nb = (W + ACC_BLOCK - 1) / ACC_BLOCK;
    const size_t bm_words64 = (size_t)((n + 63) / 64);
    const uint32_t bmw = (uint32_t)bm_words64;
    const uint32_t bnb = (bmw + BM_THREADS - 1) / BM_THREADS;
    if ((rc = grow(S.cnt, (size_t)(nb + 2) * sizeof(uint32_t)))) return rc;
    if ((rc = grow(S.cnt2, emit_cnt2_words(bmw) * sizeof(uint32_t)))) return rc;
    if ((rc = grow(S.acc, (size_t)W * sizeof(uint32_t)))) return rc;
    if ((rc = grow(S.bitmap, bm_words64 * 8))) return rc;
    if (!S.emit_done) MSIM_HIP(c, hipEventCreateWithFlags(&S.emit_done, hipEventDisableTiming));
    if (!raw_other) {
        if ((rc = ensure_words(c, g, 0, pos_hi + W + 1, false))) return rc;
        raw = g->s[0].d_raw;
    }
    const uint64_t pos_limit = (raw_other || e_limit == ~0ull) ? ~0ull : std::min<uint64_t>(pos_hi + W, e_limit);
    const uint32_t n_bins = (uint32_t)((n + BIN_VALUES - 1) >> BIN_SHIFT);
    const bool binned = n_bins <= (uint32_t)MAX_BINS;
    const uint32_t bin_cap = binned ? sample_bin_cap(n, k, p_acc) : 0u;
    if (binned) {
        if ((rc = grow(S.bins, (size_t)n_bins * BIN_SUBS * bin_cap * sizeof(uint32_t)))) return rc;
        if ((rc = grow(S.cursors, (size_t)MAX_BINS * BIN_SUBS * sizeof(uint32_t)))) return rc;
        if ((rc = grow(S.bitmap, (size_t)n_bins * BIN_WORDS * 4))) return rc;
    }
    hipLaunchKernelGGL(k_accept_count, dim3(nb), dim3(ACC_THREADS), 0, c->stream, raw, ps, W,
                       (uint32_t)(32 - bits), (uint32_t)n, S.cnt.p(), ps, binned ? S.cursors.p() : nullptr,
                       binned ? n_bins * BIN_SUBS : 0u);
    static const bool no_fold_scan = getenv("MSIM_NO_SCAN_FOLD") != nullptr;
    const uint32_t raw_counts = (binned && nb < (uint32_t)TAIL_LDS_OFFS && !no_fold_scan) ? 1u : 0u;
    if (!raw_counts) hipLaunchKernelGGL(k_scan_u32_w4, dim3(1), dim3(256), 0, c->stream, S.cnt.p(), nb);
    if (binned) {
        hipLaunchKernelGGL(k_bin_scatter, dim3((W + SPL_BLOCK - 1) / SPL_BLOCK), dim3(ACC_THREADS), 0, c->stream, raw, ps, W,
                           (uint32_t)(32 - bits), (uint32_t)n, k, S.cnt.p(), n_bins, bin_cap, S.cursors.p(), S.bins.p(), S.acc.p(),
                           ps, raw_counts);
        hipLaunchKernelGGL(k_bin_dedupe, dim3(n_bins), dim3(512), 0, c->stream, S.bins.p(), S.cursors.p(), bin_cap, S.bitmap.p(),
                           ps);
        hipLaunchKernelGGL(k_sample_tail, dim3(1), dim3(1024), 0, c->stream, raw, S.acc.p(), k, S.cnt.p(), nb, W,
                           (uint32_t)(32 - bits), (uint32_t)n, k, S.bitmap.p(), ps, raw_counts, (const PlanState *)nullptr,
                           (const SpecHdr *)nullptr, (unsigned long long)pos_limit);
    } else {
        MSIM_HIP(c, hipMemsetAsync(S.bitmap.p(), 0, bm_words64 * 8, c->stream));
        hipLaunchKernelGGL(k_accept_scatter, dim3(nb), dim3(ACC_THREADS), 0, c->stream, raw, ps, W,
                           (uint32_t)(32 - bits), (uint32_t)n, S.cnt.p(), S.acc.p());
        hipLaunchKernelGGL(k_bitmap_insert, dim3((k + 1023) / 1024), dim3(256), 0, c->stream, S.acc.p(), k, S.bitmap.p(), ps);
        hipLaunchKernelGGL(k_sample_tail, dim3(1), dim3(1024), 0, c->stream, raw, S.acc.p(), 0u, S.cnt.p(), nb, W,
                           (uint32_t)(32 - bits), (uint32_t)n, k, S.bitmap.p(), ps, 0u, (const PlanState *)nullptr,
                           (const SpecHdr *)nullptr, (unsigned long long)pos_limit);
    }
    MSIM_HIP(c, hipGetLastError());
    out.S = &S; out.W = W; out.bmw = bmw; out.bnb = bnb;
    return MSIM_OK;
}

static int prep_wait_words(Ctx *c, GpuPlan *g, uint64_t upto) {
    GpuStream &s = g->s[0];
    if (upto <= MT_N) return MSIM_OK;
    const uint32_t need = (uint32_t)((upto - MT_N + MT_CHUNK_WORDS - 1) / MT_CHUNK_WORDS);
    uint32_t &waited = g->prep_waited[g->prep_i];
    if (need <= waited) return MSIM_OK;
    for (size_t b = 0; b < s.ready_hi.size(); b++) {
        if (s.ready_hi[b] >= need) {
            MSIM_HIP(c, hipStreamWaitEvent(g->prep_stream, s.words_ev[b] ? s.words_ev[b] : s.ready_ev[b], 0));
            waited = s.ready_hi[b];
            break;
        }
    }
    return MSIM_OK;
}

static int enqueue_sample_ahead(Ctx *c, GpuPlan *g, const msim_range &r, int64_t d, uint64_t lo, uint64_t H, uint64_t e_limit,
                                Grow &grow, SampleLaunch &out, bool &took, bool grouped, uint64_t expect, uint32_t soft_half) {
    int rc;
    const uint32_t K = (uint32_t)r.k;
    const uint64_t n = (uint64_t)range_population(r, d);
    const int bits = bit_length64(n);
    const double p_acc = randbelow_acceptance((double)n);
    const double wd = big_sample_window((double)n, set_path_need((double)n, (double)K));
    if (wd >= 4.0e9) return fail(c, MSIM_ERR_UNSUPPORTED, "sample window beyond 2^32 words");
    const uint32_t W = (uint32_t)wd;
    const uint32_t F = (uint32_t)(H - lo);
    took = (W + ACC_BLOCK - 1) / ACC_BLOCK < (uint32_t)TAIL_LDS_OFFS && (F + ACC_BLOCK - 1) / ACC_BLOCK <= (uint32_t)AHEAD_MAX_HEAD_BLOCKS;
    if (!took) return MSIM_OK;
    const uint32_t a_max = F ? (uint32_t)std::min<double>((double)F, (double)F * p_acc + 16.0 * std::sqrt((double)F * p_acc * (1.0 - p_acc)) + 64.0) : 0u;
    const uint32_t k_core = K - a_max;
    g->prep_i = (g->prep_i + 1) % g->n_prep;
    if (!g->prep_streams[g->prep_i]) {
        int plo = 0, phi = 0;
        MSIM_HIP(c, hipDeviceGetStreamPriorityRange(&plo, &phi));
        const int prio = g->prep_i >= g->n_prep - g->n_prep_low ? plo : g->prep_prio > 0 ? plo : g->prep_prio < 0 ? phi : 0;
        MSIM_HIP(c, hipStreamCreateWithPriority(&g->prep_streams[g->prep_i], hipStreamNonBlocking, prio));
        if (g->seed_ev[0]) MSIM_HIP(c, hipStreamWaitEvent(g->prep_streams[g->prep_i], g->seed_ev[0], 0));
    }
    g->prep_stream = g->prep_streams[g->prep_i];
    hipStream_t ps_ = g->prep_stream;
    SampleSet &S = g->sample[g->unit++ % N_SETS];
    const uint32_t nb = (W + ACC_BLOCK - 1) / ACC_BLOCK;
    const uint32_t nbh = (F + ACC_BLOCK - 1) / ACC_BLOCK;
    const size_t bm_words64 = (size_t)((n + 63) / 64);
    const uint32_t bmw = (uint32_t)bm_words64;
    const uint32_t bnb = (bmw + BM_THREADS - 1) / BM_THREADS;
    const uint32_t n_bins = (uint32_t)((n + BIN_VALUES - 1) >> BIN_SHIFT);
    const uint32_t bin_cap = sample_bin_cap(n, K, p_acc);
    if ((rc = grow(S.cnt, (size_t)(nb + 2) * sizeof(uint32_t)))) return rc;
    if ((rc = grow(S.cnt2, emit_cnt2_words(bmw) * sizeof(uint32_t)))) return rc;
    if ((rc = grow(S.acc, (size_t)W * sizeof(uint32_t)))) return rc;
    if ((rc = grow(S.bins, (size_t)n_bins * BIN_SUBS * bin_cap * sizeof(uint32_t)))) return rc;
    if ((rc = grow(S.cursors, (size_t)MAX_BINS * BIN_SUBS * sizeof(uint32_t)))) return rc;
    if ((rc = grow(S.bitmap, std::max(bm_words64 * 8, (size_t)n_bins * BIN_WORDS * 4)))) return rc;
    if ((rc = grow(S.hcnt, (size_t)(nbh + 2) * sizeof(uint32_t)))) return rc;
    if ((rc = grow(S.hacc, ((size_t)nbh * ACC_BLOCK + 64) * sizeof(uint32_t)))) return rc;
    if (!S.ahead) MSIM_HIP(c, hipMalloc(&S.ahead, 2 * sizeof(PlanState) + sizeof(SpecHdr)));
    if (!S.emit_done) MSIM_HIP(c, hipEventCreateWithFlags(&S.emit_done, hipEventDisableTiming));
    if (!S.prep_done) MSIM_HIP(c, hipEventCreateWithFlags(&S.prep_done, hipEventDisableTiming));
    PlanState *ps_core = reinterpret_cast<PlanState *>(S.ahead), *ps_head = ps_core + 1;
    SpecHdr *hdr = reinterpret_cast<SpecHdr *>(ps_head + 1);
    if ((rc = ensure_words(c, g, 0, H + W + 1, false))) return rc;
    const uint32_t *raw = g->s[0].d_raw;
    if ((rc = prep_wait_words(c, g, H + W + 1))) return rc;
    if (S.pending) {
        if (hipEventQuery(S.wait_ev) == hipSuccess) S.pending = false;
        else { (void)hipGetLastError(); MSIM_HIP(c, hipStreamWaitEvent(ps_, S.wait_ev, 0)); }
    }
    if (!S.chain_done) MSIM_HIP(c, hipEventCreateWithFlags(&S.chain_done, hipEventDisableTiming));
    if (S.last_user == 1) MSIM_HIP(c, hipEventRecord(S.chain_done, c->stream));
    if ((S.last_user == 1 || S.last_user == 2) && hipEventQuery(S.chain_done) != hipSuccess) {
        (void)hipGetLastError();
        MSIM_HIP(c, hipStreamWaitEvent(ps_, S.chain_done, 0));
    }
    S.last_user = grouped ? 3 : 2;
    const uint32_t shift = (uint32_t)(32 - bits);
    hipLaunchKernelGGL(k_ahead_count, dim3(nb + nbh), dim3(ACC_THREADS), 0, ps_, raw, ps_core, ps_head, hdr, (unsigned long long)H,
                       (unsigned long long)lo, W, F, nb, shift, (uint32_t)n, S.cnt.p(), S.cursors.p(), n_bins * BIN_SUBS, S.hcnt.p(), S.hacc.p());
    hipLaunchKernelGGL(k_bin_scatter, dim3((W + SPL_BLOCK - 1) / SPL_BLOCK), dim3(ACC_THREADS), 0, ps_, raw, ps_core, W, shift,
                       (uint32_t)n, k_core, S.cnt.p(), n_bins, bin_cap, S.cursors.p(), S.bins.p(), S.acc.p(), ps_core, 1u);
    hipLaunchKernelGGL(k_bin_dedupe, dim3(n_bins), dim3(512), 0, ps_, S.bins.p(), S.cursors.p(), bin_cap, S.bitmap.p(), ps_core);
    MSIM_HIP(c, hipGetLastError());
    MSIM_HIP(c, hipEventRecord(S.prep_done, ps_));
    MSIM_HIP(c, hipStreamWaitEvent(c->stream, S.prep_done, 0));
    const double dups_est = (double)K * (double)K / (2.0 * (double)n);
    const uint32_t items_est = a_max + (uint32_t)(dups_est + 16.0 * std::sqrt(dups_est) + 64.0);
    const uint32_t G = std::max(1u, std::min(256u, (items_est + ACC_THREADS * FRINGE_ITEMS - 1) / (ACC_THREADS * FRINGE_ITEMS)));
    hipLaunchKernelGGL(k_ahead_fringe, dim3(G), dim3(ACC_THREADS), 0, c->stream, raw, g->d_ps, ps_core, ps_head, hdr,
                       (unsigned long long)lo, F, S.hcnt.p(), nbh, S.hacc.p(), S.acc.p(), K, k_core, shift, (uint32_t)n, S.bitmap.p(),
                       (unsigned long long)expect, soft_half);
    hipLaunchKernelGGL(k_sample_tail, dim3(1), dim3(1024), 0, c->stream, raw, S.acc.p(), k_core, S.cnt.p(), nb, W, shift, (uint32_t)n,
                       k_core, S.bitmap.p(), g->d_ps, 1u, ps_core, hdr, (unsigned long long)e_limit);
    MSIM_HIP(c, hipGetLastError());
    if (!grouped) MSIM_HIP(c, hipEventRecord(S.chain_done, c->stream));
    out.S = &S; out.W = W; out.bmw = bmw; out.bnb = bnb;
    c->t.snp_samples_ahead++;
    static const bool log_ahead = getenv("MSIM_DBG_AHEAD_LOG") != nullptr;
    if (log_ahead) fprintf(stderr, "msim: sample ahead of the chain: K %u, start in [%llu, %llu], core %u draws\n", K, (unsigned long long)lo, (unsigned long long)H, k_core);
    return MSIM_OK;
}

static int enqueue_snp_stage(Ctx *c, GpuPlan *g, Contig &ct, uint64_t K, const uint32_t *sn_index, uint64_t &pos_hi, Grow &grow,
                             uint8_t **aux8_out = nullptr, SnpDefer *defer = nullptr, uint64_t e_limit = ~0ull) {
    const msim_params &P = c->params;
    GpuStream &py = g->s[0];
    int rc;
    const double p_tv = 1.0 - std::min(1.0, (double)P.ti_lim / 9007199254740992.0);
    const double w2 = (double)K * (2.0 + 2.0 * p_tv) + 16.0 * std::sqrt(4.0 * (double)K) + 16384.0;
    if (w2 >= 4.0e9) return fail(c, MSIM_ERR_UNSUPPORTED, "SNP draw window beyond 2^32 words");
    const uint32_t W2 = (uint32_t)w2;
    const uint32_t nb2 = W2 / SNP_BLOCK2 + 2;
    SnpSet &T = g->snp[g->snp_unit++ % N_SETS];
    if ((rc = wait_if_pending(c, T.pending, T.wait_ev))) return rc;
    if ((rc = grow(T.maps, (size_t)(nb2 + 1) * sizeof(SnpMap)))) return rc;
    if (aux8_out) {
        if ((rc = grow(T.aux8, (size_t)K + 64))) return rc;
        *aux8_out = T.aux8.p();
    }
    if (!T.base) MSIM_HIP(c, hipMalloc(&T.base, 64));
    if (!T.emit_done) MSIM_HIP(c, hipEventCreateWithFlags(&T.emit_done, hipEventDisableTiming));
    if ((rc = ensure_words(c, g, 0, ((pos_hi + W2) / SNP_BLOCK2 + 2) * SNP_BLOCK2))) return rc;
    if (py.maps_ti_lim != P.ti_lim) {
        if (!py.ready_ev.empty()) MSIM_HIP(c, hipStreamWaitEvent(c->stream, py.ready_ev.back(), 0));
        if (py.mapped_blocks)
            hipLaunchKernelGGL(k_snp_maps_abs, dim3(py.mapped_blocks), dim3(SNP_THREADS), 0, c->stream, py.d_raw,
                               (uint32_t)(MT_N + (uint64_t)py.n_chunks * MT_CHUNK_WORDS), (unsigned long long)P.ti_lim, 0u, py.d_maps, py.d_lanes);
        py.maps_ti_lim = P.ti_lim;
    }
    hipLaunchKernelGGL(k_snp_scan_cut_abs, dim3(1), dim3(SNP_THREADS), 0, c->stream, py.d_lanes, g->d_ps, W2,
                       py.d_maps, T.maps.p(), nb2, (uint32_t)K, T.base,
                       (unsigned long long)(e_limit == ~0ull ? ~0ull : std::min<uint64_t>(pos_hi + W2, e_limit)));
    MSIM_HIP(c, hipGetLastError());
    if (defer) { defer->T = &T; defer->W2 = W2; defer->nb2 = nb2; }
    if (!c->chain_only && !defer) {
        hipEvent_t ce = next_chain_event(g);
        MSIM_HIP(c, hipEventRecord(ce, c->stream));
        MSIM_HIP(c, hipStreamWaitEvent(c->emit_stream, ce, 0));
        hipLaunchKernelGGL(k_snp_emit_abs, dim3(nb2), dim3(SNP_THREADS), 0, c->emit_stream, py.d_lanes, T.base, W2,
                           T.maps.p(), nb2, ct.d_recs.p(), (uint32_t)K, sn_index, aux8_out ? T.aux8.p() : (uint8_t *)nullptr);
        MSIM_HIP(c, hipGetLastError());
        if (!aux8_out) {
            MSIM_HIP(c, hipEventRecord(T.emit_done, c->emit_stream));
            T.wait_ev = T.emit_done;
            T.pending = true;
        }
    }
    pos_hi += W2;
    return MSIM_OK;
}

static void emit_train_launch(hipStream_t es, const SnpLane *lanes, EmitJobs &J, bool train3) {
    uint32_t blk = 0, eblk = 0, cblk = 0, xblk = 0;
    for (uint32_t i = 0; i < J.n; i++) {
        EmitJob &T = J.j[i];
        T.blk0 = blk; T.eblk0 = eblk; T.cblk0 = cblk; T.xblk0 = xblk;
        blk += T.bnb; eblk += T.nb2; cblk += emit_supers(T.bmw); xblk += emit_blocks(T.bmw);
    }
    J.total_blk = blk; J.total_eblk = eblk; J.total_cblk = cblk;
    if (train3) {
        if (eblk + cblk) hipLaunchKernelGGL(k_snp_emit_count_b, dim3(eblk + cblk), dim3(SNP_THREADS), 0, es, lanes, J);
        if (xblk) hipLaunchKernelGGL(k_bitmap_expand_tiles_b, dim3(xblk), dim3(BM_THREADS), 0, es, J);
    } else {
        if (blk) hipLaunchKernelGGL(k_bitmap_count_b, dim3(blk), dim3(BM_THREADS), 0, es, J);
        hipLaunchKernelGGL(k_scan_u32_b, dim3(J.n), dim3(256), 0, es, J);
        if (eblk) hipLaunchKernelGGL(k_snp_emit_abs_b, dim3(eblk), dim3(SNP_THREADS), 0, es, lanes, J);
        if (blk) hipLaunchKernelGGL(k_bitmap_expand_b, dim3(blk), dim3(BM_THREADS), 0, es, J);
    }
}

int gpu_emit_flush(Ctx *c) {
    GpuPlan *g = c->gpu;
    if (!g || g->emit_items.empty()) return MSIM_OK;
    std::vector<EmitItem> items;
    items.swap(g->emit_items);
// ... 61 lines not shown
    std::vector<uint64_t> cnt((size_t)n_jobs, 0);
    unsigned long long *d_err = nullptr;
    MSIM_HIP(c, dev.bytes(&d_err, sizeof(unsigned long long) * EMIT_G));
    EmitJobs J;
    memset(&J, 0, sizeof J);
    J.n = (uint32_t)n_jobs; J.d = d; J.tile_shift = tile_shift;
    hipStream_t es = c->emit_stream;
    for (int i = 0; i < n_jobs; i++) {
        if (!bm[i] || !n_words[i] || n_words[i] > (1u << 26) || !recs[i] || !aux8[i])
            return fail(c, MSIM_ERR_ARG, "msim_dbg_emit_train: a job without a bitmap or without room for its records");
        for (uint32_t q = 0; q < n_words[i]; q++) cnt[(size_t)i] += (uint64_t)__builtin_popcountll(bm[i][q]);
        n_recs[i] = cnt[(size_t)i];
        const uint64_t last = (uint64_t)start[i] + 64ull * n_words[i] + (uint64_t)d * cnt[(size_t)i];
        if (cnt[(size_t)i] > cap_recs[i] || last >= (1ull << 32) || len[i] >= (1ull << 32))
            return fail(c, MSIM_ERR_ARG, "msim_dbg_emit_train: more records than room, or positions beyond 2^32");
        const size_t n_tiles = (size_t)((len[i] + (1ull << tile_shift) - 1) >> tile_shift);
        const size_t sz[5] = {(size_t)n_words[i] * 8, emit_cnt2_words(n_words[i]) * sizeof(uint32_t),
                              (size_t)(cnt[(size_t)i] + 1) * sizeof(msim_record), (size_t)cnt[(size_t)i] + 1,
                              (n_tiles + 1) * sizeof(int32_t)};
        void *p[5];
        for (int q = 0; q < 5; q++) MSIM_HIP(c, dev.bytes(&p[q], sz[q]));
        MSIM_HIP(c, hipMemcpyAsync(p[0], bm[i], sz[0], hipMemcpyHostToDevice, es));
        MSIM_HIP(c, hipMemcpyAsync(p[3], aux8[i], (size_t)cnt[(size_t)i], hipMemcpyHostToDevice, es));
        MSIM_HIP(c, hipMemsetAsync(p[4], 0xee, sz[4], es));
        EmitJob &T = J.j[i];
        T.bm = static_cast<const uint64_t *>(p[0]); T.cnt2 = static_cast<uint32_t *>(p[1]);
        T.recs = static_cast<msim_record *>(p[2]); T.aux8 = static_cast<uint8_t *>(p[3]);
        T.bmw = n_words[i]; T.bnb = (n_words[i] + BM_THREADS - 1) / BM_THREADS; T.start = start[i]; T.K = (uint32_t)cnt[(size_t)i];
        if (train == 3 && first && first[i] && n_tiles) {
            T.first = static_cast<int32_t *>(p[4]); T.n_tiles = (uint32_t)n_tiles; T.err = d_err + i;
        }
    }
    emit_train_launch(es, nullptr, J, train == 3);
    MSIM_HIP(c, hipGetLastError());
    for (int i = 0; i < n_jobs; i++) {
        MSIM_HIP(c, hipMemcpyAsync(recs[i], J.j[i].recs, (size_t)cnt[(size_t)i] * sizeof(msim_record), hipMemcpyDeviceToHost, es));
        if (J.j[i].first)
            MSIM_HIP(c, hipMemcpyAsync(first[i], J.j[i].first, ((size_t)J.j[i].n_tiles + 1) * sizeof(int32_t), hipMemcpyDeviceToHost, es));
    }
    MSIM_HIP(c, wait_stream(es));
    return MSIM_OK;
}

int gpu_dbg_snp_draws(Ctx *c, const uint32_t *words, uint64_t n_words, uint64_t ti_lim, uint64_t start, uint32_t K, uint32_t aux_off,
                      uint32_t *lanes, uint32_t *maps, uint64_t *end_pos, uint32_t *flags, uint8_t *aux) {
    const uint64_t n_blocks = n_words / SNP_BLOCK2;
    if (!words || !lanes || !maps || !end_pos || !flags || !aux || !n_blocks || n_words >= (1ull << 28) || start >= n_blocks * SNP_BLOCK2 ||
        !K || K > n_words || aux_off >= 64)
        return fail(c, MSIM_ERR_ARG, "msim_dbg_snp_draws: bad argument");
    static_assert(sizeof(SnpLane) == 16 && sizeof(SnpMap) == 16, "msim_dbg_snp_draws hands both out as four uint32");
    const uint32_t W = (uint32_t)(n_blocks * SNP_BLOCK2 - start);
    const uint32_t nb = (uint32_t)(n_blocks - start / SNP_BLOCK2);
    const size_t sz_lanes = (size_t)(n_blocks + 1) * SNP_THREADS * sizeof(SnpLane), sz_maps = (size_t)(n_blocks + 1) * sizeof(SnpMap);
    const size_t sz_aux = (size_t)aux_off + K + 16;
    const size_t sz_raw = (size_t)n_words * 4, sz_win = (size_t)(nb + 1) * sizeof(SnpMap);
    DbgDev dev;
    uint32_t *d_raw; SnpLane *d_lanes; SnpMap *d_maps, *d_win; PlanState *d_ps; unsigned long long *d_base; uint8_t *d_aux;
    MSIM_HIP(c, dev.bytes(&d_raw, sz_raw)); MSIM_HIP(c, dev.bytes(&d_lanes, sz_lanes)); MSIM_HIP(c, dev.bytes(&d_maps, sz_maps));
    MSIM_HIP(c, dev.bytes(&d_win, sz_win)); MSIM_HIP(c, dev.bytes(&d_ps, sizeof(PlanState))); MSIM_HIP(c, dev.bytes(&d_base, 64));
    MSIM_HIP(c, dev.bytes(&d_aux, sz_aux));
    hipStream_t st = c->stream;
    PlanState ps;
    memset(&ps, 0, sizeof ps);
    ps.pos = ps.snp_base = start;
    MSIM_HIP(c, hipMemcpyAsync(d_raw, words, sz_raw, hipMemcpyHostToDevice, st));
    MSIM_HIP(c, hipMemcpyAsync(d_ps, &ps, sizeof ps, hipMemcpyHostToDevice, st));
    MSIM_HIP(c, hipMemsetAsync(d_lanes, 0xee, sz_lanes, st));
    MSIM_HIP(c, hipMemsetAsync(d_maps, 0xee, sz_maps, st));
    MSIM_HIP(c, hipMemsetAsync(d_win, 0, sz_win, st));
    MSIM_HIP(c, hipMemsetAsync(d_aux, 0xee, sz_aux, st));
    hipLaunchKernelGGL(k_snp_maps_abs, dim3((uint32_t)n_blocks), dim3(SNP_THREADS), 0, st, d_raw, (uint32_t)n_words,
                       (unsigned long long)ti_lim, 0u, d_maps, d_lanes);
    hipLaunchKernelGGL(k_snp_scan_cut_abs, dim3(1), dim3(SNP_THREADS), 0, st, d_lanes, d_ps, W, d_maps, d_win, nb, K, d_base, ~0ull);
    hipLaunchKernelGGL(k_snp_emit_abs, dim3(nb), dim3(SNP_THREADS), 0, st, d_lanes, d_base, W, d_win, nb,
                       (msim_record *)nullptr, K, (const uint32_t *)nullptr, d_aux + aux_off);
    MSIM_HIP(c, hipGetLastError());
    MSIM_HIP(c, hipMemcpyAsync(lanes, d_lanes, sz_lanes, hipMemcpyDeviceToHost, st));
    MSIM_HIP(c, hipMemcpyAsync(maps, d_maps, sz_maps, hipMemcpyDeviceToHost, st));
    MSIM_HIP(c, hipMemcpyAsync(aux, d_aux, sz_aux, hipMemcpyDeviceToHost, st));
    MSIM_HIP(c, hipMemcpyAsync(&ps, d_ps, sizeof ps, hipMemcpyDeviceToHost, st));
    MSIM_HIP(c, wait_stream(st));
    *end_pos = ps.pos;
    *flags = ps.flags;
    return MSIM_OK;
}

bool gpu_emit_pending(Ctx *c, int contig, bool mark_apply) {
    GpuPlan *g = c->gpu;
    if (!g) return false;
    for (EmitItem &it : g->emit_items)
        if (it.contig == contig) { if (mark_apply) it.apply = true; return true; }
    return false;
}

StreamMoments sample_words_moments(uint64_t n, uint64_t k) {
    const double n_d = (double)n, k_d = (double)k;
    const double p_acc = n_d / (double)(1ull << bit_length64(n));
    const double l1p = std::log1p(-k_d / n_d);
    const double EA = -n_d * l1p, VA = std::max(0.0, n_d * (k_d / (n_d - k_d) + l1p));
    return StreamMoments{EA / p_acc, EA * (1.0 - p_acc) / (p_acc * p_acc) + VA / (p_acc * p_acc)};
}
StreamMoments snp_words_moments(uint64_t K, unsigned long long ti_lim) {
    const double p_tv = 1.0 - std::min(1.0, (double)ti_lim / 9007199254740992.0);
    return StreamMoments{(double)K * (2.0 + 2.0 * p_tv), (double)K * (2.0 * p_tv + 4.0 * p_tv * (1.0 - p_tv))};
}

int plan_contig_gpu(Ctx *c, GpuPlan *g, Contig &ct, const msim_range *ranges, int n_ranges) {
    const msim_params &P = c->params;
    const int64_t d = min_block(P);
    int rc;
    if ((rc = session_open(c, g))) return rc;
    uint64_t K = 0;
    for (int i = 0; i < n_ranges; i++) K += (uint64_t)ranges[i].k;
    if (K >= (1ull << 31)) return fail(c, MSIM_ERR_UNSUPPORTED, "more than 2^31 mutations on one contig");
    Grow grow{c};
    if (!c->chain_only) {
        const size_t want = std::max<uint64_t>(K, 1) * sizeof(msim_record);
        if (ct.d_recs.cap < want || ct.d_pool.cap < 2 * PAD) {
            MSIM_HIP(c, wait_stream(c->stream));
            MSIM_HIP(c, wait_stream(c->emit_stream));
        }
        if ((rc = dev_reserve(c, ct.d_recs, want))) return rc;
        if ((rc = dev_reserve(c, ct.d_pool, 2 * PAD))) return rc;
    }
    ct.n_rec = K;
    ct.pool_len = 0;
    ct.plan_empty = K == 0;
    ct.all_snp = true;

    GpuStream &py = g->s[0];
    if ((rc = chain_open(c, g, true))) return rc;
    uint64_t pos_hi = py.pos;
    uint64_t rec_base = 0;
    if (c->chain_only) { g->pass_chain_only++; g->sharded_rank = true; }
    if (!g->unverified) {
        g->est_ok = true;
        g->est_e = (double)py.pos; g->est_v = 0.0; g->est_lo = py.pos;
    }
    auto est_hi = [&](uint64_t bound) -> uint64_t {
        if (!g->est_ok) return bound;
        const double m = g->est_v > 0.0 ? 16.0 * std::sqrt(1.1 * g->est_v) + 256.0 : 0.0;
        return std::min<uint64_t>(bound, (uint64_t)std::ceil(g->est_e + m));
    };
    int n_draw = 0;
    for (int i = 0; i < n_ranges; i++) n_draw += ranges[i].k != 0;
    static const bool no_fold = getenv("MSIM_NO_AUX_FOLD") != nullptr;
    const bool fold_aux = n_draw == 1 && !c->chain_only && !no_fold;
    static const bool no_group = getenv("MSIM_NO_EMIT_GROUP") != nullptr;
    const bool grouped = fold_aux && !no_group;
    const bool ahead_role = g->ahead == 2 || (g->ahead == 1 && g->sharded_rank);
    const int group = g->emit_group ? g->emit_group : (ahead_role ? 4 : 2);
    if (!g->emit_items.empty() && (!grouped || g->emit_d != (uint32_t)d || g->emit_items.size() >= (size_t)group))
        if ((rc = gpu_emit_flush(c))) return rc;
    struct { SampleSet *S; uint32_t bmw, bnb, start; } late = {nullptr, 0, 0, 0};
    for (int i = 0; i < n_ranges; i++) {
        const msim_range &r = ranges[i];
        if (r.k == 0) continue;
        const uint32_t k = (uint32_t)r.k;
        SampleLaunch sl;
        const double n_d = (double)range_population(r, d);
        const StreamMoments ms = sample_words_moments((uint64_t)n_d, (uint64_t)k);
        const double e_samp = ms.e, v_samp = ms.v;
        bool ahead = false;
        uint64_t lo = 0, H = 0, expect = 0;
        uint32_t soft_half = 0;
        if ((g->ahead == 2 || (g->ahead == 1 && g->sharded_rank)) && (grouped || (c->chain_only && n_draw == 1)) && g->est_ok && (uint64_t)n_d <= ((uint64_t)MAX_BINS << BIN_SHIFT) && 4.0 * (double)k <= n_d) {
// ... 1237 lines not shown
```

mutation-simulator_amd/csrc/plan_kernels.h:

```cpp
#pragma once
#include <algorithm>

#include "ctx.h"
#include "mt_jump_table.h"
#include "scan_kernels.h"

namespace msim {

namespace {

constexpr int GEN_STEP = MT_N - MT_M;
constexpr int JUMP_Z = MT_POLY_DEG + MT_N;
constexpr int ACC_THREADS = 256;
constexpr int ACC_ITEMS = 8;
constexpr int ACC_BLOCK = ACC_THREADS * ACC_ITEMS;
constexpr int SNP_THREADS = 256;


constexpr int BM_THREADS = 256;

enum : uint32_t { FLAG_SAMPLE_OVERFLOW = 1u, FLAG_SNP_OVERFLOW = 2u };

struct PlanState {
    unsigned long long pos;
// ... 419 lines not shown
    const uint32_t rel = (uint32_t)(s - lo);
    if (blockIdx.x == 0 && threadIdx.x == 0 && soft_half) {
        const unsigned long long dev = s > expect ? s - expect : expect - s;
        atomicMax(&ps->ahead_margin_used, (uint32_t)min(1000000ull, 1000ull * dev / soft_half));
    }
    const uint32_t blk = min(rel / ACC_BLOCK, nbh);
    uint32_t h_acc = 0, skip = 0;
    if (nbh) {
        {
            const uint32_t i0 = blk * ACC_BLOCK + threadIdx.x * ACC_ITEMS;
            uint32_t c = 0;
#pragma unroll
            for (int q = 0; q < ACC_ITEMS; q++) {
                uint32_t v;
                if (i0 + q < rel && accepted(raw, lo + i0 + q, shift, n, v)) c++;
            }
            for (int o = 32; o > 0; o >>= 1) c += __shfl_down(c, o, 64);
            if ((threadIdx.x & 63) == 0) red[threadIdx.x >> 6] = c;
            __syncthreads();
            skip = red[0] + red[1] + red[2] + red[3];
        }
        uint32_t v[4], sum = 0;
#pragma unroll
        for (int q = 0; q < 4; q++) {
            const uint32_t b = threadIdx.x * 4 + q;
            v[q] = (b >= blk && b < nbh) ? hcnt[b] - (b == blk ? skip : 0u) : 0u;
            sum += v[q];
        }
        uint32_t run = wg_scan_incl(sum, wsum) - sum;
#pragma unroll
        for (int q = 0; q < 4; q++) {
            const uint32_t b = threadIdx.x * 4 + q;
            if (b <= AHEAD_MAX_HEAD_BLOCKS) hoff[b] = run;
            run += v[q];
        }
        if (threadIdx.x == ACC_THREADS - 1) hoff[AHEAD_MAX_HEAD_BLOCKS] = run;
        __syncthreads();
        h_acc = hoff[AHEAD_MAX_HEAD_BLOCKS];
    }
    const uint32_t items = K - k_core + ps_core->dups;
    if (h_acc > items) {
        if (blockIdx.x == 0 && threadIdx.x == 0) atomicOr(&ps->flags, FLAG_SAMPLE_OVERFLOW);
        return;
    }
    if (blockIdx.x == 0 && threadIdx.x == 0) {
        hdr->need0 = items - h_acc;
        const uint32_t fl = ps_core->flags | ps_head->flags;
        if (fl) atomicOr(&ps->flags, fl);
    }
    uint32_t d = 0;
    const uint32_t stride = gridDim.x * ACC_THREADS;
    for (uint32_t base = blockIdx.x * ACC_THREADS + threadIdx.x; base < items; base += FRINGE_ITEMS * stride) {
        uint32_t old[FRINGE_ITEMS], bit[FRINGE_ITEMS];
#pragma unroll
        for (int q = 0; q < FRINGE_ITEMS; q++) {
            const uint32_t i = base + q * stride;
            old[q] = 0; bit[q] = 0;
            if (i < items) {
                uint32_t v;
                if (i < h_acc) {
                    uint32_t lo_b = blk, hi_b = nbh;
                    while (hi_b - lo_b > 1) {
                        const uint32_t mid = (lo_b + hi_b) >> 1;
                        if (hoff[mid] <= i) lo_b = mid; else hi_b = mid;
                    }
                    v = hacc[lo_b * ACC_BLOCK + (i - hoff[lo_b]) + (lo_b == blk ? skip : 0u)];
                } else {
                    v = tail[i - h_acc];
                }
                if (v < n) {
                    bit[q] = 1u << (v & 31);
                    old[q] = atomicOr(&bitmap[v >> 5], bit[q]);
                }
            }
        }
#pragma unroll
        for (int q = 0; q < FRINGE_ITEMS; q++) d += (old[q] & bit[q]) ? 1u : 0u;
    }
    for (int o = 32; o > 0; o >>= 1) d += __shfl_down(d, o, 64);
    if ((threadIdx.x & 63) == 0 && d) atomicAdd(&hdr->d1, d);
}

constexpr int TAIL_LDS_OFFS = 8192;
__global__ __launch_bounds__(1024) void k_sample_tail(const uint32_t *__restrict__ raw, const uint32_t *__restrict__ acc,
                                                      uint32_t acc_first,
                                                      const uint32_t *__restrict__ block_off, uint32_t n_blocks,
                                                      uint32_t W, uint32_t shift, uint32_t n, uint32_t k,
                                                      uint32_t *__restrict__ bitmap, PlanState *__restrict__ ps,
                                                      uint32_t raw_counts = 0, const PlanState *__restrict__ ps_win = nullptr,
                                                      const SpecHdr *__restrict__ hdr = nullptr,
                                                      unsigned long long pos_limit = ~0ull) {
    __shared__ uint32_t red[16];
    __shared__ uint32_t s_need, s_pos, s_blk, s_total;
    __shared__ uint32_t loff[TAIL_LDS_OFFS + 1];
    const bool offs_in_lds = n_blocks <= TAIL_LDS_OFFS;
    uint32_t total_acc;
    if (raw_counts) {
        uint32_t v[8], sum = 0;
#pragma unroll
        for (int q = 0; q < 8; q++) {
            const uint32_t i = threadIdx.x * 8 + q;
            v[q] = i < n_blocks ? block_off[i] : 0;
            sum += v[q];
        }
        uint32_t run = wg_scan_incl(sum, red) - sum;
#pragma unroll
        for (int q = 0; q < 8; q++) {
            const uint32_t i = threadIdx.x * 8 + q;
            if (i <= n_blocks) loff[i] = run;
            run += v[q];
        }
        if (threadIdx.x == 1023) s_total = run;
        __syncthreads();
        total_acc = s_total;
    } else {
        if (offs_in_lds)
            for (uint32_t i = threadIdx.x; i <= n_blocks; i += 1024) loff[i] = block_off[i];
        total_acc = block_off[n_blocks];
    }
    if (threadIdx.x == 0) { s_pos = hdr ? k + hdr->need0 : k; s_need = hdr ? hdr->d1 : ps->dups; }
    __syncthreads();
    if (total_acc < s_pos) {
        if (threadIdx.x == 0) atomicOr(&ps->flags, FLAG_SAMPLE_OVERFLOW);
        return;
    }
    while (true) {
        const uint32_t need = s_need, pos = s_pos;
        if (need == 0) break;
        if (pos + need > total_acc) {
            if (threadIdx.x == 0) atomicOr(&ps->flags, FLAG_SAMPLE_OVERFLOW);
            return;
        }
        uint32_t d = 0;
        for (uint32_t i = threadIdx.x; i < need; i += 1024) {
            const uint32_t v = acc[pos - acc_first + i];
            const uint32_t bit = 1u << (v & 31);
            const uint32_t old = atomicOr(&bitmap[v >> 5], bit);
            if (old & bit) d++;
        }
        for (int o = 32; o > 0; o >>= 1) d += __shfl_down(d, o, 64);
        __syncthreads();
        if ((threadIdx.x & 63) == 0) red[threadIdx.x >> 6] = d;
        __syncthreads();
        if (threadIdx.x == 0) {
            uint32_t t = 0;
            for (int w = 0; w < 16; w++) t += red[w];
            s_pos = pos + need;
            s_need = t;
        }
        __syncthreads();
    }
    const uint32_t A = s_pos;
    if (threadIdx.x == 0) {
        uint32_t lo = 0, hi = n_blocks;
        while (hi - lo > 1) {
            const uint32_t mid = (lo + hi) >> 1;
            if ((offs_in_lds ? loff[mid] : block_off[mid]) < A) lo = mid; else hi = mid;
        }
        s_blk = lo;
    }
    __syncthreads();
    const uint32_t b = s_blk;
    const uint32_t want = A - (offs_in_lds ? loff[b] : block_off[b]);
    const unsigned long long p0 = ps_win ? ps_win->pos : ps->pos;
    uint32_t f[2], v;
    const uint32_t i0 = b * ACC_BLOCK + threadIdx.x * 2;
    f[0] = (i0 < W && accepted(raw, p0 + i0, shift, n, v)) ? 1u : 0u;
// ... 1087 lines not shown
    if (i >= consumed) return;
    uint32_t lo = span[0], hi = span[1] + 1;
    while (hi - lo > 1) {
        const uint32_t mid = (lo + hi) >> 1;
        if (cut[mid] <= i) lo = mid; else hi = mid;
    }
    const WalkRange R = ranges[lo];
    if (R.pool) return;
    const uint32_t v = mt_temper(raw[*p0_slot + i]) >> __clz(R.n);
    if (v < R.n) {
        const uint32_t b = R.start + v;
        atomicOr(&bits[b >> 5], 1u << (b & 31));
    }
}

__global__ void k_advance_pos_save(PlanState *ps, unsigned long long words, unsigned long long *p0_slot) {
    *p0_slot = ps->pos;
    ps->pos += words;
    ps->snp_base = ps->pos;
}

__global__ __launch_bounds__(256) void k_list_to_bits(const uint32_t *__restrict__ list, uint32_t n, uint32_t *__restrict__ bits) {
    const uint32_t i = blockIdx.x * 256 + threadIdx.x;
    if (i >= n) return;
    const uint32_t b = list[i];
    atomicOr(&bits[b >> 5], 1u << (b & 31));
}

__global__ __launch_bounds__(BM_THREADS) void k_walk_expand(uint64_t *__restrict__ bm, uint32_t n_words,
                                                            const uint32_t *__restrict__ block_off,
                                                            const WalkRange *__restrict__ ranges, uint32_t n_ranges,
                                                            uint32_t d, msim_record *__restrict__ recs) {
    __shared__ uint32_t part[BM_THREADS];
    const uint32_t i = blockIdx.x * BM_THREADS + threadIdx.x;
    uint64_t w = i < n_words ? bm[i] : 0;
    if (w) bm[i] = 0;
    const uint32_t c = (uint32_t)__popcll(w);
    part[threadIdx.x] = c;
    __syncthreads();
    for (int o = 1; o < BM_THREADS; o <<= 1) {
        const uint32_t t = threadIdx.x >= (unsigned)o ? part[threadIdx.x - o] : 0;
        __syncthreads();
        part[threadIdx.x] += t;
        __syncthreads();
    }
    uint32_t rank = block_off[blockIdx.x] + part[threadIdx.x] - c;
    uint32_t r = 0;
    bool have = false;
    while (w) {
        const uint32_t bit = i * 64 + (uint32_t)__builtin_ctzll(w);
        w &= w - 1;
        if (!have || (r + 1 < n_ranges && ranges[r + 1].start <= bit)) {
            uint32_t lo = 0, hi = n_ranges;
            while (hi - lo > 1) {
                const uint32_t mid = (lo + hi) >> 1;
                if (ranges[mid].start <= bit) lo = mid; else hi = mid;
            }
            r = lo;
            have = true;
        }
        const uint32_t pos = bit + d * (rank - ranges[r].rec_base);
        msim_record rec;
        rec.pos = pos; rec.stop = pos; rec.extra = 0; rec.type = MSIM_SN; rec.aux = 0; rec.rsv = 0;
        recs[rank] = rec;
        rank++;
    }
}


__global__ void k_publish(const PlanState *__restrict__ ps, PlanState *__restrict__ mailbox) {
    *mailbox = *ps;
    __threadfence_system();
}

__global__ void k_publish_seq(const PlanState *__restrict__ ps, PlanState *__restrict__ mailbox,
                              uint32_t *__restrict__ seq_word, uint32_t seq) {
    *mailbox = *ps;
    __threadfence_system();
    __hip_atomic_store(seq_word, seq, __ATOMIC_RELEASE, __HIP_MEMORY_SCOPE_SYSTEM);
}

__global__ void k_raise_flag(PlanState *ps, uint32_t flag) { ps->flags |= flag; }

__global__ void k_state_init(PlanState *ps, unsigned long long pos) {
    ps->pos = pos; ps->snp_base = pos; ps->flags = 0; ps->dups = 0; ps->accepted_used = 0;
    ps->n_nsn = ps->n_rec = ps->n_sn = ps->pool_len = 0;
    ps->len_delta = 0;
    ps->ahead_margin_used = 0; ps->rsv = 0;
}

}

}
```

mutation-simulator_amd/mutation_simulator_amd/_ffi.py:

```python
from __future__ import annotations

import ctypes as C
import os
from pathlib import Path

import numpy as np

PKG_DIR = Path(__file__).resolve().parent
LIB_CANDIDATES = [PKG_DIR.parent / "lib" / "libmsim.so"]

OK, ERR_ARG, ERR_HIP, ERR_VALUE, ERR_KEY, ERR_UNSUPPORTED, ERR_NOMEM, ERR_IO = range(8)
PLAN_AUTO, PLAN_HOST, PLAN_GPU = 0, 1, 2
RNG_FAST = 4


class MsimError(RuntimeError):
    code = None


class MsimUnsupported(MsimError):
    """Valid for the reference, outside this build's scope (translocations, >= 4 GiB contigs)."""


class Record(C.Structure):
# ... 57 lines not shown
    C.POINTER(C.c_uint32), C.POINTER(C.c_int)
SYMBOLS = [
    ("msim_abi_version", C.c_int, []),
    ("msim_warm_up", C.c_int, [C.c_int]),
    ("msim_create", C.c_int, [C.c_int, C.c_uint32, C.POINTER(_VP)]),
    ("msim_destroy", None, [_VP]),
    ("msim_last_error", C.c_char_p, [_VP]),
    ("msim_device_name", C.c_int, [_VP, C.c_char_p, C.c_int]),
    ("msim_sync", C.c_int, [_VP]),
    ("msim_set_plan_mode", C.c_int, [_VP, C.c_uint32]),
    ("msim_seed", C.c_int, [_VP, _U32P, C.c_int, C.c_uint32]),
    ("msim_set_mt_state", C.c_int, [_VP, C.c_int, _U32P, C.c_int]),
    ("msim_get_mt_state", C.c_int, [_VP, C.c_int, _U32P, _IP]),
    ("msim_reserve_streams", C.c_int, [_VP, C.c_uint64, C.c_uint64]),
    ("msim_add_contig", C.c_int, [_VP, _VP, C.c_uint64, _IP]),
    ("msim_add_contig_synthetic", C.c_int, [_VP, C.c_uint64, C.c_uint64, _IP]),
    ("msim_contig_length", C.c_int, [_VP, C.c_int, _U64P]),
    ("msim_read_contig", C.c_int, [_VP, C.c_int, C.c_uint64, C.c_uint64, _VP]),
    ("msim_clear", C.c_int, [_VP]),
    ("msim_set_params", C.c_int, [_VP, C.POINTER(Params)]),
    ("msim_plan_contig", C.c_int, [_VP, C.c_int, C.POINTER(Range), C.c_int]),
    ("msim_plan_chain", C.c_int, [_VP, C.c_uint64, C.POINTER(Range), C.c_int]),
    ("msim_plan_was_empty", C.c_int, [_VP, C.c_int, _IP]),
    ("msim_apply_contig", C.c_int, [_VP, C.c_int]),
    ("msim_key_error", C.c_int, [_VP, C.c_int, _U8P, _U64P]),
    ("msim_result_sizes", C.c_int, [_VP, C.c_int, _U64P, _U64P, _U64P]),
    ("msim_fetch_sequence", C.c_int, [_VP, C.c_int, C.c_uint64, C.c_uint64, _VP]),
    ("msim_fetch_records", C.c_int, [_VP, C.c_int, _VP, _VP]),
    ("msim_result_checksum", C.c_int, [_VP, C.c_int, _U64P]),
    ("msim_release_result", C.c_int, [_VP, C.c_int]),
    ("msim_result_device_ptr", C.c_int, [_VP, C.c_int, _U64P, _U64P]),
    ("msim_render_vcf", C.c_int, [_VP, C.c_uint64, _VP, _VP, C.c_uint64, C.c_char_p, _VP,
                                  C.c_uint64, _U64P]),
    ("msim_render_vcf_gt", C.c_int, [_VP, _VP, C.c_uint64, _VP, _VP, C.c_uint64, C.c_char_p, _VP, C.c_uint64, _U64P]),
    ("msim_genotype_contig", C.c_int, [_VP, C.c_int, C.c_uint64, C.c_uint32, C.c_uint64]),
    ("msim_set_genotypes", C.c_int, [_VP, C.c_int, _VP]),
    ("msim_fetch_genotypes", C.c_int, [_VP, C.c_int, _VP]),
    ("msim_select_haplotype", C.c_int, [_VP, C.c_int, C.c_int]),
    ("msim_render_chain", C.c_int, [_VP, C.c_uint64, C.c_uint64, C.c_char_p, C.c_char_p, C.c_uint64, _VP, C.c_uint64, _U64P]),
    ("msim_render_chain_device", C.c_int, [_VP, C.c_int, C.c_char_p, C.c_char_p, C.c_uint64, _VP, C.c_uint64, _U64P]),
    ("msim_render_vcf_device", C.c_int, [_VP, C.c_int, C.c_char_p, _VP, C.c_uint64, _U64P]),
    ("msim_fetch_sequence_framed", C.c_int, [_VP, C.c_int, C.c_uint32, _VP, C.c_uint64, _U64P]),
    ("msim_render_vcf_device_file", C.c_int, [_VP, C.c_int, C.c_char_p, C.c_int, C.c_uint64, _U64P]),
    ("msim_fetch_sequence_framed_file", C.c_int, [_VP, C.c_int, C.c_uint32, C.c_int, C.c_uint64, _U64P]),
    ("msim_file_wait", C.c_int, [_VP]),
    ("msim_bgzf_open", C.c_int, [_VP, C.c_int, C.c_int]),
    ("msim_bgzf_append", C.c_int, [_VP, C.c_int, _VP, C.c_uint64]),
    ("msim_bgzf_close", C.c_int, [_VP, C.c_int, _U64P, _U64P]),
    ("msim_bgzf_bound", C.c_uint64, [C.c_uint64]),
    ("msim_bgzf_compress", C.c_int, [_VP, _VP, C.c_uint64, _VP, C.c_uint64, _U64P, C.POINTER(C.c_float)]),
    ("msim_bgzf_probe", C.c_int, [_VP, C.c_uint64, _U64P, _U64P]),
    ("msim_bgzf_inflate", C.c_int, [_VP, _VP, C.c_uint64, _VP, C.c_uint64, _U64P, C.POINTER(C.c_float)]),
    ("msim_vcf_load", C.c_int, [_VP, _VP, C.c_uint64, _U64P, _U64P]),
    ("msim_vcf_groups", C.c_int, [_VP, _VP, C.c_uint64, _U64P]),
    ("msim_vcf_select", C.c_int, [_VP, C.c_uint32, C.c_uint32, C.c_uint32]),
    ("msim_vcf_plan_contig", C.c_int, [_VP, C.c_int, C.c_int64]),
    ("msim_vcf_host_bases", C.c_int, [_VP, C.c_int, _VP]),
    ("msim_vcf_timing", C.c_int, [_VP, C.POINTER(C.c_double), C.POINTER(C.c_double)]),
    ("msim_vcf_release", C.c_int, [_VP]),
    ("msim_device_host_cpus", C.c_int, [C.c_int, C.c_char_p, C.c_int]),
    ("msim_batch_fetch_file", C.c_int, [_VP, C.c_int, C.c_uint64, C.c_int, C.c_uint64]),
    ("msim_add_contig_text", C.c_int, [_VP, _VP, C.c_uint64, C.c_uint64, C.c_uint32, C.c_uint32, _IP]),
    ("msim_splice_contigs", C.c_int, [_VP, C.c_int, C.c_int, C.c_uint64, _U64P, _U64P, _IP]),
    ("msim_set_fast_key", C.c_int, [_VP, C.c_uint64]),
    ("msim_sample_min_distance", C.c_int, [_VP, C.c_int64, C.c_int64, C.c_int64, C.c_int64, C.c_int64, _VP]),
    ("msim_host_alloc", C.c_int, [_VP, C.c_uint64, C.POINTER(_VP)]),
    ("msim_host_free", C.c_int, [_VP, _VP]),
    ("msim_batch_run", C.c_int, [_VP, C.POINTER(BatchContig), C.c_int]),
    ("msim_batch_sizes", C.c_int, [_VP, C.c_int, _U64P, _U64P, C.POINTER(C.c_int32), _U64P]),
    ("msim_batch_fetch", C.c_int, [_VP, _VP, C.c_uint64, _VP, C.c_uint64]),
    ("msim_batch_view", C.c_int, [_VP, C.POINTER(C.c_void_p), _U64P, C.POINTER(C.c_void_p), _U64P, _U64P]),
    ("msim_batch_key_contig", C.c_int, [_VP, _IP]),
    ("msim_fasta_index", C.c_int, [_VP, C.c_uint64, _VP, C.c_uint64, _U64P]),
    ("msim_build_ranges", C.c_int, [_VP, C.c_int, _VP, _VP, _VP, C.c_int64, _VP]),
    ("msim_comm_unique_id", C.c_int, [_VP]),
    ("msim_comm_init", C.c_int, [_VP, _VP, C.c_int, C.c_int]),
    ("msim_comm_destroy", C.c_int, [_VP]),
    ("msim_planned_out_len", C.c_int, [_VP, C.c_int, _U64P, _IP]),
    ("msim_gather_to_root", C.c_int, [_VP, C.c_int, _IP, _IP, _U64P, _U64P, _U64P, C.c_int, _U64P]),
    ("msim_gather_plan", C.c_int, [C.c_int, _IP, _U64P, _U64P, _U64P, C.c_int, C.c_int, C.c_int, C.POINTER(C.c_int64), _IP]),
    ("msim_gather_fetch", C.c_int, [_VP, C.c_uint64, C.c_uint64, _VP]),
    ("msim_dbg_snp_draws", C.c_int, [_VP, _VP, C.c_uint64, C.c_uint64, C.c_uint64, C.c_uint32, C.c_uint32, _VP, _VP, _U64P,
                                     _U32P, _VP]),
    ("msim_context_counts", C.c_int, [_VP, C.c_int, _VP, _U64P]),
    ("msim_plan_contig_spectrum", C.c_int, [_VP, C.c_int, _VP, C.c_uint64, C.c_uint32]),
    ("msim_spectrum_timing", C.c_int, [_VP, C.POINTER(C.c_double), C.POINTER(C.c_double)]),
    ("msim_dbg_context_counts", C.c_int, [_VP, C.c_uint64, _VP, _U64P]),
    ("msim_dbg_spectrum_plan", C.c_int, [_VP, C.c_uint64, _VP, C.c_uint64, C.c_uint32, _VP, C.c_uint64, _U64P]),
    ("msim_sbs_counts", C.c_int, [_VP, C.c_int, _VP, _VP]),
    ("msim_sbs_timing", C.c_int, [_VP, C.POINTER(C.c_double)]),
    ("msim_dbg_sbs_counts", C.c_int, [_VP, C.c_uint64, _VP, C.c_uint64, _VP, _VP]),
    ("msim_cmp_hold", C.c_int, [_VP, C.c_int]),
    ("msim_cmp_release", C.c_int, [_VP, C.c_int]),
    ("msim_cmp_counts", C.c_int, [_VP, C.c_int, C.c_uint32, _VP, _VP]),
    ("msim_cmp_fetch", C.c_int, [_VP, C.c_int, _U64P, _U64P, _VP, _VP, _VP, _VP]),
    ("msim_cmp_timing", C.c_int, [_VP, C.POINTER(C.c_double)]),
    ("msim_dbg_cmp_counts", C.c_int, [_VP, C.c_uint64, _VP, C.c_uint64, _VP, C.c_uint64, _VP, C.c_uint64, _VP, C.c_uint64,
                                      C.c_uint32, _VP, _VP, _VP, _VP]),
    ("msim_cmp_counts_blocks", C.c_int, [_VP, C.c_int, C.c_uint32, C.c_uint32, _VP, _VP, _VP]),
    ("msim_cmp_blocks_timing", C.c_int, [_VP, C.POINTER(C.c_double)]),
    ("msim_dbg_cmp_counts_blocks", C.c_int, [_VP, C.c_uint64, _VP, C.c_uint64, _VP, C.c_uint64, _VP, C.c_uint64, _VP, C.c_uint64,
                                             C.c_uint32, C.c_uint32, _VP, _VP, _VP, _VP, _VP]),
    ("msim_cmp_join", C.c_int, [_VP, C.c_int, C.c_int]),
    ("msim_cmp_counts_diploid", C.c_int, [_VP, C.c_int, C.c_uint32, _VP, _VP]),
    ("msim_cmp_fetch_diploid", C.c_int, [_VP, C.c_int, C.c_int, _U64P, _U64P, _VP, _VP, _VP, _VP]),
    ("msim_cmp_join_timing", C.c_int, [_VP, C.POINTER(C.c_double)]),
    ("msim_dbg_cmp_join", C.c_int, [_VP, C.c_uint64, _VP, C.c_uint64, _VP, C.c_uint64, _VP, C.c_uint64, _VP, _VP, _VP, _U64P]),
    ("msim_dbg_cmp_counts_diploid", C.c_int, [_VP, C.c_uint64, _VP, C.c_uint64, _VP, C.c_uint64, _VP, _VP, C.c_uint64, _VP,
                                              C.c_uint64, _VP, C.c_uint32, _VP, _VP, _VP, _VP]),
    ("msim_stats", C.c_int, [_VP, C.POINTER(Timing)]),
    ("msim_reset_stats", C.c_int, [_VP]),
]
CMP_EXACT = 1
CMP_BINS = 5
CMP_PASS = 256
CMP_WINDOW = 65536
CMP_BLOCK_GAP = 50
CMP_BLOCK_RECORDS, CMP_BLOCK_SPAN = 64, 4096
CMP_TRUTH, CMP_CALLS = 0, 1
CMP_JOIN_TILE = 1024
SPECTRUM_TILE = 4096
SBS_CHANNELS, SBS_TALLIES = 96, 8
SBS_PASS = 1024

_lib = None


def library_path() -> Path:
    env = os.environ.get("MSIM_LIB")
    if env:
        return Path(env)
    for p in LIB_CANDIDATES:
        if p.exists():
            return p
    raise MsimError(
        f"libmsim.so not found (looked in {[str(p) for p in LIB_CANDIDATES]}); build it with "
        "`make -C mutation-simulator_amd/csrc` or `python -c 'import __graft_entry__ as g; g.build()'`")


def load():
    global _lib
    if _lib is None:
        lib = C.CDLL(str(library_path()))
        for name, restype, argtypes in SYMBOLS:
            fn = getattr(lib, name)
            fn.restype = restype
            fn.argtypes = argtypes
        if lib.msim_abi_version() != 8:
            raise MsimError("libmsim ABI version mismatch")
        _lib = lib
    return _lib


def render_chain(recs: np.ndarray, length: int, t_name: str, q_name: str, chain_id: int) -> bytes:
    lib = load()
    recs = np.ascontiguousarray(recs, dtype=RECORD_DTYPE)
    t, q = t_name.encode("utf-8", "replace"), q_name.encode("utf-8", "replace")
    need = C.c_uint64()
    rc = lib.msim_render_chain(_ptr(recs), len(recs), int(length), t, q, int(chain_id), None, 0, C.byref(need))
    if rc != OK:
        raise MsimError(f"msim_render_chain failed ({rc})")
    out = np.empty(need.value, dtype=np.uint8)
    if need.value:
        rc = lib.msim_render_chain(_ptr(recs), len(recs), int(length), t, q, int(chain_id), _ptr(out), need.value, C.byref(need))
        if rc != OK:
            raise MsimError(f"msim_render_chain failed ({rc})")
    return out.tobytes()


TYPE_TABLE_DTYPE = np.dtype([("thr", "<u8", (8,)), ("n", "<u4"), ("type", "u1", (8,)), ("_pad", "u1", (4,))])
MIX_RANGE_DTYPE = np.dtype([("rec_base", "<u4"), ("clip", "<u4"), ("set_id", "<u4"), ("rsv", "<u4")])
CHAIN_DROPPED = 0xFFFFFFFF
CHAIN_TOMBSTONE = 0x80


def chain_lg_rows(n_classes: int) -> int:
    return 0 if n_classes <= 1 else 1 if n_classes == 2 else 2 if n_classes <= 4 else 3


def accept_tables_host(tempered, classes) -> np.ndarray:
    fn = load().msim_dbg_accept_tables_host
    fn.restype, fn.argtypes = C.c_int, [_VP, C.c_uint32, _VP, _VP, C.c_uint32, _VP]
    words = np.ascontiguousarray(tempered, dtype=np.uint32)
    sh = np.array([c[0] for c in classes], dtype=np.uint32)
    width = np.array([c[1] for c in classes], dtype=np.uint32)
    T = np.full((len(words) + 1, 1 << chain_lg_rows(len(classes))), 0xdddddddd, dtype=np.uint32)
    rc = fn(_ptr(words), len(words), _ptr(sh), _ptr(width), len(classes), _ptr(T))
    if rc != OK:
        err = MsimError(f"msim_dbg_accept_tables_host failed ({rc})")
        err.code = rc
        raise err
    return T


def chain_tile() -> int:
    fn = load().msim_dbg_chain_tile
    fn.restype, fn.argtypes = C.c_uint32, []
    return int(fn())


def parse_cpulist(text: str) -> set:
    out = set()
    for part in text.strip().split(","):
        if not part:
            continue
        a, _, b = part.partition("-")
        out.update(range(int(a), int(b or a) + 1))
    return out


def warm_up_async(device: int = 0, pin: bool = False):
    import threading
    lib = load()
    caller = threading.get_native_id()

    def work():
        lib.msim_warm_up(int(device))
        if not pin or os.environ.get("MSIM_NO_PIN") == "1" or not hasattr(os, "sched_setaffinity"):
            return
        try:
            buf = C.create_string_buffer(4096)
            if lib.msim_device_host_cpus(int(device), buf, 4096) != OK or not buf.value:
                return
            cpus = parse_cpulist(buf.value.decode()) & os.sched_getaffinity(caller)
            if cpus:
                os.sched_setaffinity(caller, cpus)
        except (OSError, ValueError):
            pass
    t = threading.Thread(target=work, name="msim-warm-up", daemon=True)
    t.start()
    return t


def _ptr(a: np.ndarray):
    return C.c_void_p(a.ctypes.data)


class Engine:

    def __init__(self, device: int = 0, flags: int = PLAN_AUTO):
        self.lib = load()
        self.h = C.c_void_p()
        if flags == PLAN_AUTO and os.environ.get("MSIM_PLAN_MODE"):
            flags = int(os.environ["MSIM_PLAN_MODE"])
        rc = self.lib.msim_create(device, flags, C.byref(self.h))
        if rc != OK:
            msg = self.lib.msim_last_error(None).decode()
            self.h = None
            raise MsimError(f"msim_create failed ({rc}): {msg}")
        self._pinned: list = []

    def close(self):
        if getattr(self, "h", None):
            for p in getattr(self, "_pinned", []):
# ... 290 lines not shown
    def cmp_counts_blocks(self, contig: int, exact: bool = False, gap: int = CMP_BLOCK_GAP) -> tuple:
        counts = np.zeros((8, CMP_BINS, 6), dtype=np.uint64)
        tallies = np.zeros(2, dtype=np.uint64)
        blocks = np.zeros(5, dtype=np.uint64)
        self._check(self.lib.msim_cmp_counts_blocks(self.h, int(contig), CMP_EXACT if exact else 0, int(gap), _ptr(counts),
                                                    _ptr(tallies), _ptr(blocks)), contig)
        return counts, tallies, blocks

    def cmp_blocks_timing(self) -> float:
        a = C.c_double()
        self._check(self.lib.msim_cmp_blocks_timing(self.h, C.byref(a)))
        return a.value

    def cmp_join(self, contig: int, side: int):
        self._check(self.lib.msim_cmp_join(self.h, int(contig), int(side)), contig)

    def cmp_counts_diploid(self, contig: int, exact: bool = False) -> tuple:
        return self._cmp_counts(self.lib.msim_cmp_counts_diploid, 6, contig, exact)

    def cmp_fetch_diploid(self, contig: int, side: int, flags: bool = True) -> tuple:
        n, m = C.c_uint64(), C.c_uint64()
        self._check(self.lib.msim_cmp_fetch_diploid(self.h, int(contig), int(side), C.byref(n), C.byref(m), None, None, None, None),
                    contig)
        recs = np.zeros(n.value, dtype=RECORD_DTYPE)
        pool = np.zeros(m.value, dtype=np.uint8)
        gt = np.zeros(n.value, dtype=np.uint8)
        fl = np.zeros(n.value, dtype=np.uint8) if flags else None
        self._check(self.lib.msim_cmp_fetch_diploid(self.h, int(contig), int(side), None, None, _ptr(recs), _ptr(pool), _ptr(gt),
                                                    _ptr(fl) if flags else None), contig)
        return recs, pool, gt, fl

    def cmp_join_timing(self) -> float:
        a = C.c_double()
        self._check(self.lib.msim_cmp_join_timing(self.h, C.byref(a)))
        return a.value

    def set_records(self, contig: int, recs: np.ndarray, pool: np.ndarray, with_offsets: bool = False):
        fn = self.lib.msim_dbg_set_records
        fn.restype, fn.argtypes = C.c_int, [_VP, C.c_int, _VP, C.c_uint64, _VP, C.c_uint64, C.c_uint32]
        recs = np.ascontiguousarray(recs, dtype=RECORD_DTYPE)
        pool = np.ascontiguousarray(pool, dtype=np.uint8)
        self._check(fn(self.h, contig, _ptr(recs), len(recs), _ptr(pool), len(pool), 1 if with_offsets else 0), contig)

    def apply_batch(self, contigs):
        fn = self.lib.msim_dbg_apply_batch
        fn.restype, fn.argtypes = C.c_int, [_VP, _IP, C.c_int]
        ids = (C.c_int * len(contigs))(*[int(i) for i in contigs])
        self._check(fn(self.h, ids, len(contigs)))

    def emit_train(self, jobs, d: int = 1, train: int = 3):
        fn = self.lib.msim_dbg_emit_train
        fn.restype = C.c_int
        fn.argtypes = [_VP, C.c_int, _VP, _VP, _VP, _VP, _VP, C.c_uint32, C.c_int, _VP, _VP, _VP, _VP]
        self.lib.msim_dbg_apply_tile.restype = C.c_uint32
        tile = int(self.lib.msim_dbg_apply_tile())
        n = len(jobs)
        bms = [np.ascontiguousarray(j[0], dtype=np.uint64) for j in jobs]
        auxs = [np.ascontiguousarray(j[3], dtype=np.uint8) for j in jobs]
        caps = [max(1, int(a.shape[0])) for a in auxs]
        auxs = [a if a.shape[0] else np.zeros(1, dtype=np.uint8) for a in auxs]
        recs = [np.zeros(cap, dtype=RECORD_DTYPE) for cap in caps]
        ptrs = lambda arrs: (C.c_void_p * n)(*[a.ctypes.data for a in arrs])
        n_words = np.array([b.shape[0] for b in bms], dtype=np.uint32)
        start = np.array([int(j[1]) for j in jobs], dtype=np.uint32)
        length = np.array([int(j[2]) for j in jobs], dtype=np.uint64)
        cap_a = np.array(caps, dtype=np.uint64)
        n_recs = np.zeros(n, dtype=np.uint64)
        n_tiles = [(int(j[2]) + tile - 1) // tile for j in jobs]
        firsts = [np.zeros(nt + 1, dtype=np.int32) for nt in n_tiles] if train == 3 else None
        self._check(fn(self.h, n, ptrs(bms), _ptr(n_words), _ptr(start), _ptr(length), ptrs(auxs), int(d), int(train),
                       ptrs(recs), _ptr(cap_a), _ptr(n_recs), ptrs(firsts) if firsts else None))
        return tile, [(recs[i][:int(n_recs[i])], firsts[i] if firsts and n_tiles[i] else None) for i in range(n)]

    def snp_draws(self, words, ti_lim: int, start: int, K: int, aux_off: int = 0):
        words = np.ascontiguousarray(words, dtype=np.uint32)
        n_blocks = words.shape[0] // 8192
        lanes = np.zeros((n_blocks + 1, 256, 4), dtype=np.uint32)
        maps = np.zeros((n_blocks + 1, 4), dtype=np.uint32)
        aux = np.zeros(int(aux_off) + int(K) + 16, dtype=np.uint8)
        end_pos, flags = C.c_uint64(0), C.c_uint32(0)
        self._check(self.lib.msim_dbg_snp_draws(self.h, _ptr(words), words.shape[0], int(ti_lim), int(start), int(K), int(aux_off),
                                                _ptr(lanes), _ptr(maps), C.byref(end_pos), C.byref(flags), _ptr(aux)))
        return {"lanes": lanes, "maps": maps, "end_pos": int(end_pos.value), "flags": int(flags.value), "aux": aux}

    def candidates(self, np_words, sets, bitmap=None, start: int = 0, d: int = 1, K: int = 0, ranges=None, all: bool = False):
        fn = self.lib.msim_dbg_candidates
        fn.restype = C.c_int
        fn.argtypes = [_VP, _VP, C.c_uint32, C.c_uint32, C.c_uint32, C.c_uint32, _VP, C.c_uint32, _VP, C.c_uint32, _VP, C.c_uint64,
                       C.c_uint32, _VP, _VP, _VP, _VP, _VP, C.c_uint64, _U32P, _U32P]
        words = np.ascontiguousarray(np_words, dtype=np.uint32)
        sets = np.ascontiguousarray(np.atleast_1d(sets), dtype=TYPE_TABLE_DTYPE)
        if bitmap is not None:
            bm = np.ascontiguousarray(bitmap, dtype=np.uint64)
            cap = int(np.unpackbits(bm.view(np.uint8)).sum())
            rt, n_draw = None, 0
        else:
            bm, cap = None, int(K)
            rt = np.ascontiguousarray(ranges, dtype=MIX_RANGE_DTYPE)
            n_draw = len(rt)
        room = max(cap, 1)
        cand_pos, nsn_pos, nsn_rank = (np.zeros(room, dtype=np.uint32) for _ in range(3))
        cand_type, nsn_type = (np.zeros(room, dtype=np.uint8) for _ in range(2))
        k_out, n_nsn = C.c_uint32(), C.c_uint32()
        self._check(fn(self.h, _ptr(bm) if bm is not None else None, len(bm) if bm is not None else 0, int(start), int(d), int(K),
                       _ptr(rt) if rt is not None else None, n_draw, _ptr(sets), len(sets), _ptr(words), len(words), 1 if all else 0,
                       _ptr(cand_pos), _ptr(cand_type), _ptr(nsn_pos), _ptr(nsn_type), _ptr(nsn_rank), cap, C.byref(k_out),
                       C.byref(n_nsn)))
        k, m = k_out.value, n_nsn.value
        return {"cand_pos": cand_pos[:k] if bm is not None else None, "cand_type": cand_type[:k],
                "nsn_pos": nsn_pos[:m] if bm is not None else None, "nsn_type": nsn_type[:m], "nsn_rank": nsn_rank[:m], "n_nsn": m}

    def accept_tables(self, raw_words, n: int, p0: int, classes):
        fn = self.lib.msim_dbg_accept_tables
        fn.restype, fn.argtypes = C.c_int, [_VP, _VP, C.c_uint64, C.c_uint64, C.c_uint32, _VP, _VP, C.c_uint32, _VP, _VP]
        words = np.ascontiguousarray(raw_words, dtype=np.uint32)
        sh = np.array([c[0] for c in classes], dtype=np.uint32)
        width = np.array([c[1] for c in classes], dtype=np.uint32)
        rows = 1 << chain_lg_rows(len(classes))
        T = np.full((int(n) + 1, rows), 0xdddddddd, dtype=np.uint32)
        T_ps = np.full((int(n) + 1, rows), 0xdddddddd, dtype=np.uint32)
        self._check(fn(self.h, _ptr(words), len(words), int(p0), int(n), _ptr(sh), _ptr(width), len(classes), _ptr(T), _ptr(T_ps)))
        return T, T_ps

    def mixed_emit(self, length: int, cand_pos, cand_type, ch_rank, ch_stop, np_words, ch_extra=None, ch_aux=None, ranges=None,
                   visit_from=None, sn_chained: bool = False):
        fn = self.lib.msim_dbg_mixed_emit
        fn.restype = C.c_int
        fn.argtypes = [_VP, C.c_uint64, C.c_uint32, _VP, _VP, C.c_uint32, _VP, _VP, _VP, _VP, C.c_uint32, _VP, _VP, C.c_uint32, _VP,
                       C.c_uint64, _VP, _VP, _VP, _VP, C.c_uint64, _VP, C.POINTER(C.c_int64)]
        pos = np.ascontiguousarray(cand_pos, dtype=np.uint32)
        typ = np.ascontiguousarray(cand_type, dtype=np.uint8)
        rank = np.ascontiguousarray(ch_rank, dtype=np.uint32)
        stop = np.ascontiguousarray(ch_stop, dtype=np.uint32)
        words = np.ascontiguousarray(np_words, dtype=np.uint32)
        extra = None if ch_extra is None else np.ascontiguousarray(ch_extra, dtype=np.uint32)
        aux = None if ch_aux is None else np.ascontiguousarray(ch_aux, dtype=np.uint8)
        rt = None if ranges is None else np.ascontiguousarray(ranges, dtype=MIX_RANGE_DTYPE)
        visit = None if visit_from is None else np.ascontiguousarray(visit_from, dtype=np.uint32)
        k = len(pos)
        assert len(typ) == k and len(stop) == len(rank)
        opt = lambda a: _ptr(a) if a is not None else None
        recs = np.zeros(max(k, 1), dtype=RECORD_DTYPE)
        rec_off, sn_index = np.zeros(max(k, 1), dtype=np.uint32), np.zeros(max(k, 1), dtype=np.uint32)
        cap_pool = len(words)
        pool = np.zeros(max(cap_pool, 1), dtype=np.uint8)
        counts = np.zeros(4, dtype=np.uint32)
        delta = C.c_int64()
        self._check(fn(self.h, int(length), k, _ptr(pos), _ptr(typ), len(rank), _ptr(rank), _ptr(stop), opt(extra), opt(aux),
                       0 if rt is None else len(rt), opt(rt), opt(visit), 1 if sn_chained else 0, _ptr(words), len(words), _ptr(recs),
                       _ptr(rec_off), _ptr(sn_index), _ptr(pool), cap_pool, _ptr(counts), C.byref(delta)))
        n_rec, n_sn, pool_len = (int(x) for x in counts[:3])
        return {"recs": recs[:n_rec], "rec_off": rec_off[:n_rec], "sn_index": sn_index[:n_sn], "pool": pool[:pool_len],
                "n_rec": n_rec, "n_sn": n_sn, "pool_len": pool_len, "len_delta": int(delta.value)}

    def key_error(self, contig: int):
        base, pos = C.c_uint8(), C.c_uint64()
        rc = self.lib.msim_sync(self.h)
        if rc not in (OK, ERR_KEY):
            self._check(rc, contig)
        if self.lib.msim_key_error(self.h, contig, C.byref(base), C.byref(pos)) != OK:
            return None
        return chr(base.value), pos.value

    def render_vcf_device(self, contig: int, seq_name: str, guess: int = 0) -> np.ndarray:
        need = C.c_uint64()
        name = seq_name.encode("utf-8", "replace")
# ... 475 lines not shown
```

Baseline: 919,800.

## Seed generator states via kernel arguments and overlap error-count copies with plan finish

Replaces the per-stream pinned host staging and two H2D memcpys per generator with a single k_reseed kernel that takes the Mersenne Twister state as a by-value argument and also initialises the plan state, merging both streams under one event. In the non-fast drain path, the apply error/delta copies are enqueued on the emit stream before the plan-finish sync, so a separate later round trip is avoided. It also adds a debug entry point for k_sample_tail and names its thread count as a constant. The main risk is the large kernel argument of MT_N words (about 2.5 KB), and the emit-stream wait now always runs in apply_finish.

```diff
diff --git a/include/msim.h b/include/msim.h
--- a/include/msim.h
+++ b/include/msim.h
@@ -288,6 +288,12 @@
 int msim_dbg_snp_draws(msim_ctx *ctx, const uint32_t *words, uint64_t n_words, uint64_t ti_lim, uint64_t start, uint32_t K,
                        uint32_t aux_off, uint32_t *lanes, uint32_t *maps, uint64_t *end_pos, uint32_t *flags, uint8_t *aux);
 
+typedef struct msim_dbg_tail_state { uint64_t pos, snp_base; uint32_t flags, dups, accepted_used, rsv; } msim_dbg_tail_state;
+int msim_dbg_sample_tail(msim_ctx *ctx, const uint32_t *words, uint64_t n_words, const uint32_t *acc, uint64_t n_acc,
+                         uint32_t acc_first, const uint32_t *blocks, uint32_t n_blocks, uint32_t raw_counts, uint32_t W,
+                         uint32_t shift, uint32_t n, uint32_t k, uint32_t *bitmap, uint32_t bm_guard, msim_dbg_tail_state *state,
+                         int anchored, uint64_t win_pos, uint32_t need0, uint32_t d1, uint64_t pos_limit);
+
 int msim_stats(msim_ctx *ctx, msim_timing *out);
 int msim_reset_stats(msim_ctx *ctx);
 
diff --git a/mutation-simulator_amd/csrc/apply.hip b/mutation-simulator_amd/csrc/apply.hip
--- a/mutation-simulator_amd/csrc/apply.hip
+++ b/mutation-simulator_amd/csrc/apply.hip
@@ -852,8 +852,22 @@
     return MSIM_OK;
 }
 
+int apply_ride_err_copies(Ctx *c) {
+    if (c->fast || c->pending_apply.empty() || c->errs_riding) return MSIM_OK;
+    for (int idx : c->pending_apply) {
+        if (idx < 0 || (size_t)idx >= c->contigs.size()) continue;
+        const hipStream_t s = c->contigs[(size_t)idx].apply_stream;
+        if (s && s != c->emit_stream) return MSIM_OK;
+    }
+    const int rc = enqueue_err_copies(c);
+    if (rc) return rc;
+    c->errs_riding = true;
+    return MSIM_OK;
+}
+
 int apply_finish(Ctx *c) {
-    bool have_errs = false;
+    bool have_errs = c->errs_riding;
+    c->errs_riding = false;
     {
         int state = 0;
         const bool ride = c->fast && !c->pending_apply.empty();
@@ -872,7 +886,7 @@
         }
         const int rc = fast_plan_collect(c, ride ? enqueue_err_copies : nullptr, &state);
         if (rc) { c->pending_apply.clear(); for (auto &g : c->contigs) g.apply_pending = g.dyn_applied = false; return rc; }
-        have_errs = state == 1;
+        have_errs = have_errs || state == 1;
     }
     if (c->pending_apply.empty()) return MSIM_OK;
     {
@@ -887,8 +901,8 @@
     if (!have_errs) {
         const int rc = enqueue_err_copies(c);
         if (rc) return rc;
-        MSIM_HIP(c, wait_stream(c->emit_stream));
-    }
+    }
+    MSIM_HIP(c, wait_stream(c->emit_stream));
     unsigned long long *errs = c->h_errs.p(), *deltas = c->h_errs.p() + nc;
     bool delta_mismatch = false;
     hipEvent_t origin = nullptr;
diff --git a/mutation-simulator_amd/csrc/ctx.h b/mutation-simulator_amd/csrc/ctx.h
--- a/mutation-simulator_amd/csrc/ctx.h
+++ b/mutation-simulator_amd/csrc/ctx.h
@@ -108,6 +108,7 @@
     Pinned<unsigned long long> h_mail;
     Scratch<unsigned long long> d_errs;
     Pinned<unsigned long long> h_errs;
+    bool errs_riding = false;
     std::vector<int> pending_apply;
     Scratch<uint8_t> d_text;
     uint64_t text_len = 0;
@@ -340,6 +341,7 @@
 int apply_contig_device(Ctx *c, Contig &g);
 int apply_batch_device(Ctx *c, const std::vector<int> &ids, bool batch_rewrites);
 int apply_finish(Ctx *c);
+int apply_ride_err_copies(Ctx *c);
 uint32_t apply_tile_shift();
 int apply_prepare_tile_index(Ctx *c, Contig &g, hipStream_t st, int32_t **first, uint32_t *n_tiles, uint32_t *tile_shift,
                              unsigned long long **err);
diff --git a/mutation-simulator_amd/csrc/msim_api.hip b/mutation-simulator_amd/csrc/msim_api.hip
--- a/mutation-simulator_amd/csrc/msim_api.hip
+++ b/mutation-simulator_amd/csrc/msim_api.hip
@@ -90,7 +90,7 @@
 static int drain(Ctx *c) {
     if (c->host_only) return MSIM_OK;
     TraceRange tr("msim drain (collect deferred results)");
-    int rc = c->gpu ? gpu_plan_finish(c, c->gpu) : MSIM_OK;
+    int rc = c->gpu ? gpu_plan_finish(c, c->gpu, true) : MSIM_OK;
     int rc2 = apply_finish(c);
     if (rc) return rc;
     if (rc2) return rc2;
@@ -1397,6 +1397,19 @@
     return gpu_dbg_snp_draws(c, words, n_words, ti_lim, start, K, aux_off, lanes, maps, end_pos, flags, aux);
 }
 
+int msim_dbg_sample_tail(msim_ctx *p, const uint32_t *words, uint64_t n_words, const uint32_t *acc, uint64_t n_acc, uint32_t acc_first,
+                         const uint32_t *blocks, uint32_t n_blocks, uint32_t raw_counts, uint32_t W, uint32_t shift, uint32_t n,
+                         uint32_t k, uint32_t *bitmap, uint32_t bm_guard, msim_dbg_tail_state *state, int anchored, uint64_t win_pos,
+                         uint32_t need0, uint32_t d1, uint64_t pos_limit) {
+    CTX_FLUSHED(c, p)
+    if (!c) return MSIM_ERR_ARG;
+    NEED_GPU(c);
+    int rc = drain(c);
+    if (rc) return rc;
+    return gpu_dbg_sample_tail(c, words, n_words, acc, n_acc, acc_first, blocks, n_blocks, raw_counts, W, shift, n, k, bitmap, bm_guard,
+                               state, anchored, win_pos, need0, d1, pos_limit);
+}
+
 int msim_dbg_candidates(msim_ctx *p, const uint64_t *bitmap, uint32_t n_words, uint32_t start, uint32_t d, uint32_t K,
                         const void *rt, uint32_t n_draw, const void *sets, uint32_t n_sets, const uint32_t *np_words, uint64_t n_np_words,
                         uint32_t all, uint32_t *cand_pos, uint8_t *cand_type, uint32_t *nsn_pos, uint8_t *nsn_type, uint32_t *nsn_rank,
diff --git a/mutation-simulator_amd/csrc/plan_gpu.h b/mutation-simulator_amd/csrc/plan_gpu.h
--- a/mutation-simulator_amd/csrc/plan_gpu.h
+++ b/mutation-simulator_amd/csrc/plan_gpu.h
@@ -10,7 +10,7 @@
 void gpu_plan_invalidate(GpuPlan *g);
 int gpu_plan_sync_to_host(Ctx *c, GpuPlan *g);
 void gpu_plan_reserve(GpuPlan *g, uint64_t py_words, uint64_t np_words);
-int gpu_plan_finish(Ctx *c, GpuPlan *g);
+int gpu_plan_finish(Ctx *c, GpuPlan *g, bool ride_errs = false);
 bool gpu_plan_eligible(const Ctx *c, const msim_range *ranges, int n_ranges);
 int plan_contig_gpu(Ctx *c, GpuPlan *g, Contig &ct, const msim_range *ranges, int n_ranges);
 bool gpu_plan_mixed_eligible(const Ctx *c, const msim_range *ranges, int n_ranges);
@@ -26,6 +26,10 @@
                        msim_record *const *recs, const uint64_t *cap_recs, uint64_t *n_recs, int32_t *const *first);
 int gpu_dbg_snp_draws(Ctx *c, const uint32_t *words, uint64_t n_words, uint64_t ti_lim, uint64_t start, uint32_t K, uint32_t aux_off,
                       uint32_t *lanes, uint32_t *maps, uint64_t *end_pos, uint32_t *flags, uint8_t *aux);
+int gpu_dbg_sample_tail(Ctx *c, const uint32_t *words, uint64_t n_words, const uint32_t *acc, uint64_t n_acc, uint32_t acc_first,
+                        const uint32_t *blocks, uint32_t n_blocks, uint32_t raw_counts, uint32_t W, uint32_t shift, uint32_t n,
+                        uint32_t k, uint32_t *bitmap, uint32_t bm_guard, msim_dbg_tail_state *state, int anchored, uint64_t win_pos,
+                        uint32_t need0, uint32_t d1, uint64_t pos_limit);
 int gpu_dbg_candidates(Ctx *c, const uint64_t *bm, uint32_t n_words, uint32_t start, uint32_t d, uint32_t K, const void *rt,
                        uint32_t n_draw, const void *sets, uint32_t n_sets, const uint32_t *np_raw, uint64_t n_np, uint32_t all,
                        uint32_t *cand_pos, uint8_t *cand_type, uint32_t *nsn_pos, uint8_t *nsn_type, uint32_t *nsn_rank, uint64_t cap,
diff --git a/mutation-simulator_amd/csrc/plan_gpu.hip b/mutation-simulator_amd/csrc/plan_gpu.hip
--- a/mutation-simulator_amd/csrc/plan_gpu.hip
+++ b/mutation-simulator_amd/csrc/plan_gpu.hip
@@ -119,8 +119,7 @@
     Staging<uint8_t> h_naux;
     MixSets mm_sets;
     const msim_range *mm_for = nullptr; int mm_n = 0;
-    uint32_t *h_seed = nullptr;
-    hipEvent_t seed_ev[2] = {nullptr, nullptr};
+    hipEvent_t seed_ev = nullptr;
     hipStream_t gen_stream = nullptr;
     hipStream_t jump_stream = nullptr;
     std::vector<hipEvent_t> ev_pool;
@@ -294,8 +293,7 @@
     for (auto e : g->grp_ev) if (e) (void)hipEventDestroy(e);
     if (g->t0) (void)hipEventDestroy(g->t0);
     if (g->t1) (void)hipEventDestroy(g->t1);
-    if (g->h_seed) (void)hipHostFree(g->h_seed);
-    for (auto e : g->seed_ev) if (e) (void)hipEventDestroy(e);
+    if (g->seed_ev) (void)hipEventDestroy(g->seed_ev);
     if (g->d_poly) (void)hipFree(g->d_poly);
     if (g->d_ps) (void)hipFree(g->d_ps);
     if (g->h_mail) (void)hipHostFree(g->h_mail);
@@ -580,18 +578,21 @@
     return MSIM_OK;
 }
 
-static int stream_to_device(Ctx *c, GpuPlan *g, int si) {
-    GpuStream &s = g->s[si];
-    HostMT &h = si ? c->np : c->py;
-    if (s.live) return MSIM_OK;
-    if (!s.d_states) {
-        MSIM_HIP(c, hipMalloc(&s.d_states, (size_t)MT_N * sizeof(uint32_t)));
-        s.states_cap = 1;
-    }
-    if (!s.d_raw) {
-        MSIM_HIP(c, hipMalloc(&s.d_raw, (size_t)MT_N * sizeof(uint32_t)));
-        s.cap = MT_N;
-    }
+static int streams_to_device(Ctx *c, GpuPlan *g) {
+    if (g->s[0].live && g->s[1].live) return MSIM_OK;
+    for (int si = 0; si < 2; si++) {
+        GpuStream &s = g->s[si];
+        if (s.live) continue;
+        if (!s.d_states) {
+            MSIM_HIP(c, hipMalloc(&s.d_states, (size_t)MT_N * sizeof(uint32_t)));
+            s.states_cap = 1;
+        }
+        if (!s.d_raw) {
+            MSIM_HIP(c, hipMalloc(&s.d_raw, (size_t)MT_N * sizeof(uint32_t)));
+            s.cap = MT_N;
+        }
+    }
+    if (!g->d_ps) MSIM_HIP(c, hipMalloc(&g->d_ps, sizeof(PlanState)));
     {
         int rc0 = ensure_side_streams(c, g);
         if (rc0) return rc0;
@@ -599,44 +600,52 @@
     MSIM_HIP(c, wait_stream(g->jump_stream));
     MSIM_HIP(c, wait_stream(g->gen_stream));
     for (auto st : g->prep_streams) if (st) MSIM_HIP(c, wait_stream(st));
-    if (!g->h_seed) MSIM_HIP(c, hipHostMalloc(&g->h_seed, 2 * sizeof h.mt, hipHostMallocDefault));
-    if (!g->seed_ev[si]) MSIM_HIP(c, hipEventCreateWithFlags(&g->seed_ev[si], hipEventDisableTiming));
-    else MSIM_HIP(c, wait_event(g->seed_ev[si]));
-    uint32_t *slot = g->h_seed + (size_t)si * MT_N;
-    memcpy(slot, h.mt, sizeof h.mt);
-    MSIM_HIP(c, hipMemcpyAsync(s.d_states, slot, sizeof h.mt, hipMemcpyHostToDevice, c->stream));
-    MSIM_HIP(c, hipMemcpyAsync(s.d_raw, slot, sizeof h.mt, hipMemcpyHostToDevice, c->stream));
-    MSIM_HIP(c, hipEventRecord(g->seed_ev[si], c->stream));
-    MSIM_HIP(c, hipStreamWaitEvent(g->jump_stream, g->seed_ev[si], 0));
-    MSIM_HIP(c, hipStreamWaitEvent(g->gen_stream, g->seed_ev[si], 0));
-    if (si == 0) for (auto st : g->prep_streams) if (st) MSIM_HIP(c, hipStreamWaitEvent(st, g->seed_ev[si], 0));
-    for (auto e : s.ready_ev) g->ev_pool.push_back(e);
-    s.ready_ev.clear();
-    s.ready_hi.clear();
-    for (auto e : s.words_ev) if (e) g->ev_pool.push_back(e);
-    s.words_ev.clear();
-    s.waited_chunks = 0;
-    s.waited_words = 0;
-    if (si == 0) for (auto &w : g->prep_waited) w = 0;
-    s.casc_pending = false;
-    s.n_states = 1;
-    s.lvl = 0; s.n_src = 1; s.m_done = 0;
-    s.z_lvl = -1;
-    s.n_chunks = 0;
-    s.mapped_blocks = 0;
-    s.maps_ti_lim = c->params.ti_lim;
-    s.pos = (uint64_t)h.idx;
-    s.max_upto = 0;
-    s.live = true;
-    if (si == 0) { g->ps_valid = false; g->verified_pos = s.pos; }
+    if (!g->seed_ev) MSIM_HIP(c, hipEventCreateWithFlags(&g->seed_ev, hipEventDisableTiming));
+    static_assert(sizeof(SeedWords) == sizeof(HostMT::mt), "k_reseed carries a host generator's state words");
+    for (int si = 0; si < 2; si++) {
+        GpuStream &s = g->s[si];
+        if (s.live) continue;
+        HostMT &h = si ? c->np : c->py;
+        SeedWords sw;
+        memcpy(sw.w, h.mt, sizeof sw.w);
+        hipLaunchKernelGGL(k_reseed, dim3(1), dim3(256), 0, c->stream, sw, s.d_states, s.d_raw, si == 0 ? g->d_ps : (PlanState *)nullptr,
+                           (unsigned long long)h.idx);
+        MSIM_HIP(c, hipGetLastError());
+    }
+    MSIM_HIP(c, hipEventRecord(g->seed_ev, c->stream));
+    MSIM_HIP(c, hipStreamWaitEvent(g->jump_stream, g->seed_ev, 0));
+    MSIM_HIP(c, hipStreamWaitEvent(g->gen_stream, g->seed_ev, 0));
+    for (auto st : g->prep_streams) if (st) MSIM_HIP(c, hipStreamWaitEvent(st, g->seed_ev, 0));
+    for (int si = 0; si < 2; si++) {
+        GpuStream &s = g->s[si];
+        if (s.live) continue;
+        HostMT &h = si ? c->np : c->py;
+        for (auto e : s.ready_ev) g->ev_pool.push_back(e);
+        s.ready_ev.clear();
+        s.ready_hi.clear();
+        for (auto e : s.words_ev) if (e) g->ev_pool.push_back(e);
+        s.words_ev.clear();
+        s.waited_chunks = 0;
+        s.waited_words = 0;
+        if (si == 0) for (auto &w : g->prep_waited) w = 0;
+        s.casc_pending = false;
+        s.n_states = 1;
+        s.lvl = 0; s.n_src = 1; s.m_done = 0;
+        s.z_lvl = -1;
+        s.n_chunks = 0;
+        s.mapped_blocks = 0;
+        s.maps_ti_lim = c->params.ti_lim;
+        s.pos = (uint64_t)h.idx;
+        s.max_upto = 0;
+        s.live = true;
+        if (si == 0) { g->ps_valid = true; g->verified_pos = s.pos; }
+    }
     return MSIM_OK;
 }
 
 static int session_open(Ctx *c, GpuPlan *g) {
     int rc;
-    if ((rc = stream_to_device(c, g, 0))) return rc;
-    if ((rc = stream_to_device(c, g, 1))) return rc;
-    if (!g->d_ps) MSIM_HIP(c, hipMalloc(&g->d_ps, sizeof(PlanState)));
+    if ((rc = streams_to_device(c, g))) return rc;
     if (!g->h_mail) MSIM_HIP(c, hipHostMalloc(&g->h_mail, sizeof(PlanState), hipHostMallocMapped));
     return MSIM_OK;
 }
@@ -696,7 +705,7 @@
     return true;
 }
 
-int gpu_plan_finish(Ctx *c, GpuPlan *g) {
+int gpu_plan_finish(Ctx *c, GpuPlan *g, bool ride_errs) {
     {
         const int rc = gpu_emit_flush(c);
         if (rc) return rc;
@@ -705,6 +714,10 @@
     hipLaunchKernelGGL(k_publish, dim3(1), dim3(1), 0, c->stream, g->d_ps, g->h_mail);
     MSIM_HIP(c, hipGetLastError());
     MSIM_HIP(c, hipEventRecord(g->t1, c->stream));
+    if (ride_errs) {
+        const int rc = apply_ride_err_copies(c);
+        if (rc) return rc;
+    }
     MSIM_HIP(c, wait_stream(c->stream));
     MSIM_HIP(c, wait_stream(c->emit_stream));
     float ms = 0;
@@ -813,7 +826,7 @@
                            ps, raw_counts);
         hipLaunchKernelGGL(k_bin_dedupe, dim3(n_bins), dim3(512), 0, c->stream, S.bins.p(), S.cursors.p(), bin_cap, S.bitmap.p(),
                            ps);
-        hipLaunchKernelGGL(k_sample_tail, dim3(1), dim3(1024), 0, c->stream, raw, S.acc.p(), k, S.cnt.p(), nb, W,
+        hipLaunchKernelGGL(k_sample_tail, dim3(1), dim3(TAIL_THREADS), 0, c->stream, raw, S.acc.p(), k, S.cnt.p(), nb, W,
                            (uint32_t)(32 - bits), (uint32_t)n, k, S.bitmap.p(), ps, raw_counts, (const PlanState *)nullptr,
                            (const SpecHdr *)nullptr, (unsigned long long)pos_limit);
     } else {
@@ -821,7 +834,7 @@
         hipLaunchKernelGGL(k_accept_scatter, dim3(nb), dim3(ACC_THREADS), 0, c->stream, raw, ps, W,
                            (uint32_t)(32 - bits), (uint32_t)n, S.cnt.p(), S.acc.p());
         hipLaunchKernelGGL(k_bitmap_insert, dim3((k + 1023) / 1024), dim3(256), 0, c->stream, S.acc.p(), k, S.bitmap.p(), ps);
-        hipLaunchKernelGGL(k_sample_tail, dim3(1), dim3(1024), 0, c->stream, raw, S.acc.p(), 0u, S.cnt.p(), nb, W,
+        hipLaunchKernelGGL(k_sample_tail, dim3(1), dim3(TAIL_THREADS), 0, c->stream, raw, S.acc.p(), 0u, S.cnt.p(), nb, W,
                            (uint32_t)(32 - bits), (uint32_t)n, k, S.bitmap.p(), ps, 0u, (const PlanState *)nullptr,
                            (const SpecHdr *)nullptr, (unsigned long long)pos_limit);
     }
@@ -867,7 +880,7 @@
         MSIM_HIP(c, hipDeviceGetStreamPriorityRange(&plo, &phi));
         const int prio = g->prep_i >= g->n_prep - g->n_prep_low ? plo : g->prep_prio > 0 ? plo : g->prep_prio < 0 ? phi : 0;
         MSIM_HIP(c, hipStreamCreateWithPriority(&g->prep_streams[g->prep_i], hipStreamNonBlocking, prio));
-        if (g->seed_ev[0]) MSIM_HIP(c, hipStreamWaitEvent(g->prep_streams[g->prep_i], g->seed_ev[0], 0));
+        if (g->seed_ev) MSIM_HIP(c, hipStreamWaitEvent(g->prep_streams[g->prep_i], g->seed_ev, 0));
     }
     g->prep_stream = g->prep_streams[g->prep_i];
     hipStream_t ps_ = g->prep_stream;
@@ -921,7 +934,7 @@
     hipLaunchKernelGGL(k_ahead_fringe, dim3(G), dim3(ACC_THREADS), 0, c->stream, raw, g->d_ps, ps_core, ps_head, hdr,
                        (unsigned long long)lo, F, S.hcnt.p(), nbh, S.hacc.p(), S.acc.p(), K, k_core, shift, (uint32_t)n, S.bitmap.p(),
                        (unsigned long long)expect, soft_half);
-    hipLaunchKernelGGL(k_sample_tail, dim3(1), dim3(1024), 0, c->stream, raw, S.acc.p(), k_core, S.cnt.p(), nb, W, shift, (uint32_t)n,
+    hipLaunchKernelGGL(k_sample_tail, dim3(1), dim3(TAIL_THREADS), 0, c->stream, raw, S.acc.p(), k_core, S.cnt.p(), nb, W, shift, (uint32_t)n,
                        k_core, S.bitmap.p(), g->d_ps, 1u, ps_core, hdr, (unsigned long long)e_limit);
     MSIM_HIP(c, hipGetLastError());
     if (!grouped) MSIM_HIP(c, hipEventRecord(S.chain_done, c->stream));
@@ -1149,6 +1162,54 @@
     MSIM_HIP(c, wait_stream(st));
     *end_pos = ps.pos;
     *flags = ps.flags;
+    return MSIM_OK;
+}
+
+int gpu_dbg_sample_tail(Ctx *c, const uint32_t *words, uint64_t n_words, const uint32_t *acc, uint64_t n_acc, uint32_t acc_first,
+                        const uint32_t *blocks, uint32_t n_blocks, uint32_t raw_counts, uint32_t W, uint32_t shift, uint32_t n,
+                        uint32_t k, uint32_t *bitmap, uint32_t bm_guard, msim_dbg_tail_state *state, int anchored, uint64_t win_pos,
+                        uint32_t need0, uint32_t d1, uint64_t pos_limit) {
+    if (!words || !acc || !blocks || !bitmap || !state || !n_blocks || !W || !n || shift >= 32 || n_words >= (1ull << 31) ||
+        n_blocks != (W + ACC_BLOCK - 1) / ACC_BLOCK || (raw_counts && n_blocks > (uint32_t)TAIL_LDS_OFFS) || raw_counts > 1)
+        return fail(c, MSIM_ERR_ARG, "msim_dbg_sample_tail: bad argument");
+    const uint64_t p0 = anchored ? win_pos : state->pos;
+    uint64_t total = 0;
+    if (raw_counts) for (uint32_t i = 0; i < n_blocks; i++) total += blocks[i];
+    else total = blocks[n_blocks];
+    const uint64_t first_pos = (uint64_t)k + (anchored ? need0 : 0u);
+    if (p0 > n_words || W > n_words - p0 || total >= (1ull << 32) || acc_first > first_pos || total > (uint64_t)acc_first + n_acc)
+        return fail(c, MSIM_ERR_ARG, "msim_dbg_sample_tail: the window or the list does not cover what the kernel may read");
+    for (uint64_t i = 0; i < n_acc; i++)
+        if (acc[i] >= n) return fail(c, MSIM_ERR_ARG, "msim_dbg_sample_tail: a list entry beyond the population");
+    const size_t bm_words = ((size_t)n + 31) / 32, sz_bm = (bm_words + 2 * (size_t)bm_guard) * 4;
+    const size_t sz_raw = std::max<size_t>((size_t)n_words * 4, 4), sz_acc = std::max<size_t>((size_t)n_acc * 4, 4);
+    const size_t sz_blk = ((size_t)n_blocks + 1) * 4;
+    DbgDev dev;
+    uint32_t *d_raw, *d_acc, *d_blk, *d_bm; PlanState *d_ps; SpecHdr *d_hdr;
+    MSIM_HIP(c, dev.bytes(&d_raw, sz_raw)); MSIM_HIP(c, dev.bytes(&d_acc, sz_acc)); MSIM_HIP(c, dev.bytes(&d_blk, sz_blk));
+    MSIM_HIP(c, dev.bytes(&d_bm, sz_bm)); MSIM_HIP(c, dev.bytes(&d_ps, 2 * sizeof(PlanState))); MSIM_HIP(c, dev.bytes(&d_hdr, sizeof(SpecHdr)));
+    hipStream_t st = c->stream;
+    PlanState ps[2];
+    memset(ps, 0, sizeof ps);
+    ps[0].pos = state->pos; ps[0].snp_base = state->snp_base; ps[0].flags = state->flags; ps[0].dups = state->dups;
+    ps[0].accepted_used = state->accepted_used;
+    ps[1].pos = ps[1].snp_base = win_pos;
+    SpecHdr hdr{need0, d1, 0, 0};
+    MSIM_HIP(c, hipMemcpyAsync(d_raw, words, (size_t)n_words * 4, hipMemcpyHostToDevice, st));
+    if (n_acc) MSIM_HIP(c, hipMemcpyAsync(d_acc, acc, (size_t)n_acc * 4, hipMemcpyHostToDevice, st));
+    MSIM_HIP(c, hipMemcpyAsync(d_blk, blocks, ((size_t)n_blocks + (raw_counts ? 0 : 1)) * 4, hipMemcpyHostToDevice, st));
+    MSIM_HIP(c, hipMemcpyAsync(d_bm, bitmap, sz_bm, hipMemcpyHostToDevice, st));
+    MSIM_HIP(c, hipMemcpyAsync(d_ps, ps, sizeof ps, hipMemcpyHostToDevice, st));
+    MSIM_HIP(c, hipMemcpyAsync(d_hdr, &hdr, sizeof hdr, hipMemcpyHostToDevice, st));
+    hipLaunchKernelGGL(k_sample_tail, dim3(1), dim3(TAIL_THREADS), 0, st, d_raw, d_acc, acc_first, d_blk, n_blocks, W, shift, n, k,
+                       d_bm + bm_guard, d_ps, raw_counts, anchored ? (const PlanState *)(d_ps + 1) : (const PlanState *)nullptr,
+                       anchored ? (const SpecHdr *)d_hdr : (const SpecHdr *)nullptr, (unsigned long long)pos_limit);
+    MSIM_HIP(c, hipGetLastError());
+    MSIM_HIP(c, hipMemcpyAsync(bitmap, d_bm, sz_bm, hipMemcpyDeviceToHost, st));
+    MSIM_HIP(c, hipMemcpyAsync(ps, d_ps, sizeof(PlanState), hipMemcpyDeviceToHost, st));
+    MSIM_HIP(c, wait_stream(st));
+    state->pos = ps[0].pos; state->snp_base = ps[0].snp_base; state->flags = ps[0].flags; state->dups = ps[0].dups;
+    state->accepted_used = ps[0].accepted_used;
     return MSIM_OK;
 }
 
diff --git a/mutation-simulator_amd/csrc/plan_kernels.h b/mutation-simulator_amd/csrc/plan_kernels.h
--- a/mutation-simulator_amd/csrc/plan_kernels.h
+++ b/mutation-simulator_amd/csrc/plan_kernels.h
@@ -525,7 +525,8 @@
 }
 
 constexpr int TAIL_LDS_OFFS = 8192;
-__global__ __launch_bounds__(1024) void k_sample_tail(const uint32_t *__restrict__ raw, const uint32_t *__restrict__ acc,
+constexpr int TAIL_THREADS = 1024;
+__global__ __launch_bounds__(TAIL_THREADS) void k_sample_tail(const uint32_t *__restrict__ raw, const uint32_t *__restrict__ acc,
                                                       uint32_t acc_first,
                                                       const uint32_t *__restrict__ block_off, uint32_t n_blocks,
                                                       uint32_t W, uint32_t shift, uint32_t n, uint32_t k,
@@ -1779,13 +1780,21 @@
 
 __global__ void k_raise_flag(PlanState *ps, uint32_t flag) { ps->flags |= flag; }
 
-__global__ void k_state_init(PlanState *ps, unsigned long long pos) {
+__device__ __forceinline__ void state_init(PlanState *ps, unsigned long long pos) {
     ps->pos = pos; ps->snp_base = pos; ps->flags = 0; ps->dups = 0; ps->accepted_used = 0;
     ps->n_nsn = ps->n_rec = ps->n_sn = ps->pool_len = 0;
     ps->len_delta = 0;
     ps->ahead_margin_used = 0; ps->rsv = 0;
 }
-
-}
-
-}
+__global__ void k_state_init(PlanState *ps, unsigned long long pos) { state_init(ps, pos); }
+
+struct SeedWords { uint32_t w[MT_N]; };
+__global__ __launch_bounds__(256) void k_reseed(SeedWords sw, uint32_t *__restrict__ states, uint32_t *__restrict__ raw,
+                                                PlanState *ps, unsigned long long pos) {
+    for (int i = threadIdx.x; i < MT_N; i += 256) { const uint32_t v = sw.w[i]; states[i] = v; raw[i] = v; }
+    if (ps && threadIdx.x == 0) state_init(ps, pos);
+}
+
+}
+
+}
diff --git a/mutation-simulator_amd/mutation_simulator_amd/_ffi.py b/mutation-simulator_amd/mutation_simulator_amd/_ffi.py
--- a/mutation-simulator_amd/mutation_simulator_amd/_ffi.py
+++ b/mutation-simulator_amd/mutation_simulator_amd/_ffi.py
@@ -163,6 +163,9 @@
     ("msim_gather_fetch", C.c_int, [_VP, C.c_uint64, C.c_uint64, _VP]),
     ("msim_dbg_snp_draws", C.c_int, [_VP, _VP, C.c_uint64, C.c_uint64, C.c_uint64, C.c_uint32, C.c_uint32, _VP, _VP, _U64P,
                                      _U32P, _VP]),
+    ("msim_dbg_sample_tail", C.c_int, [_VP, _VP, C.c_uint64, _VP, C.c_uint64, C.c_uint32, _VP, C.c_uint32, C.c_uint32, C.c_uint32,
+                                       C.c_uint32, C.c_uint32, C.c_uint32, _VP, C.c_uint32, _VP, C.c_int, C.c_uint64, C.c_uint32,
+                                       C.c_uint32, C.c_uint64]),
     ("msim_context_counts", C.c_int, [_VP, C.c_int, _VP, _U64P]),
     ("msim_plan_contig_spectrum", C.c_int, [_VP, C.c_int, _VP, C.c_uint64, C.c_uint32]),
     ("msim_spectrum_timing", C.c_int, [_VP, C.POINTER(C.c_double), C.POINTER(C.c_double)]),
@@ -251,6 +254,8 @@
 
 TYPE_TABLE_DTYPE = np.dtype([("thr", "<u8", (8,)), ("n", "<u4"), ("type", "u1", (8,)), ("_pad", "u1", (4,))])
 MIX_RANGE_DTYPE = np.dtype([("rec_base", "<u4"), ("clip", "<u4"), ("set_id", "<u4"), ("rsv", "<u4")])
+TAIL_STATE_DTYPE = np.dtype([("pos", "<u8"), ("snp_base", "<u8"), ("flags", "<u4"), ("dups", "<u4"), ("accepted_used", "<u4"),
+                             ("rsv", "<u4")])
 CHAIN_DROPPED = 0xFFFFFFFF
 CHAIN_TOMBSTONE = 0x80
 
@@ -707,6 +712,25 @@
         self._check(self.lib.msim_dbg_snp_draws(self.h, _ptr(words), words.shape[0], int(ti_lim), int(start), int(K), int(aux_off),
                                                 _ptr(lanes), _ptr(maps), C.byref(end_pos), C.byref(flags), _ptr(aux)))
         return {"lanes": lanes, "maps": maps, "end_pos": int(end_pos.value), "flags": int(flags.value), "aux": aux}
+
+    def sample_tail(self, words, acc, acc_first: int, blocks, raw_counts: bool, W: int, shift: int, n: int, k: int, bitmap,
+                    state: dict, win=None, pos_limit: int = 2 ** 64 - 1, guard: int = 4):
+        words = np.ascontiguousarray(words, dtype=np.uint32)
+        acc = np.ascontiguousarray(acc, dtype=np.uint32)
+        blocks = np.ascontiguousarray(blocks, dtype=np.uint32)
+        bm = np.concatenate([np.full(guard, 0xEEEEEEEE, dtype=np.uint32), np.ascontiguousarray(bitmap, dtype=np.uint32),
+                             np.full(guard, 0xEEEEEEEE, dtype=np.uint32)])
+        assert bm.shape[0] == 2 * guard + (int(n) + 31) // 32, "bitmap: ceil(n / 32) words"
+        n_blocks = blocks.shape[0] - (0 if raw_counts else 1)
+        st = np.zeros(1, dtype=TAIL_STATE_DTYPE)
+        for f in ("pos", "snp_base", "flags", "dups", "accepted_used"):
+            st[f] = int(state.get(f, 0))
+        wpos, need0, d1 = win if win is not None else (0, 0, 0)
+        self._check(self.lib.msim_dbg_sample_tail(self.h, _ptr(words), words.shape[0], _ptr(acc), acc.shape[0], int(acc_first),
+                                                  _ptr(blocks), int(n_blocks), 1 if raw_counts else 0, int(W), int(shift), int(n),
+                                                  int(k), _ptr(bm), int(guard), _ptr(st), 0 if win is None else 1, int(wpos),
+                                                  int(need0), int(d1), int(pos_limit)))
+        return {f: int(st[f][0]) for f in ("pos", "snp_base", "flags", "dups", "accepted_used")}, bm
 
     def candidates(self, np_words, sets, bitmap=None, start: int = 0, d: int = 1, K: int = 0, ranges=None, all: bool = False):
         fn = self.lib.msim_dbg_candidates
```

New measurement: 977,000 (median of 6 runs). 6.2% higher.
